# franciscotln/cosmology-model-fit

Hardware: AMD Instinct MI355X
Metric: walker-logL evals/s, Pantheon+ 1701-SN full-cov chi2, theta resident in HBM (higher is better)
Workload: dtype f64; 1 GPU; Pantheon+-shaped 1701-SN full-cov flat-LCDM chi2 + prior, 4096 walkers per GPU per step (BASELINE configs[1] at N=1), G=4000, theta resident in HBM; workload_key=pantheon, walkers_per_gpu=4096, walkers_total=4096, n_sn=1701, n_grid=4000, ndim=4, parallelism=walkers sharded over 1 GPU(s)

## Files before the change

cosmology-model-fit_amd/_lib.py:

```python
from __future__ import annotations

import ctypes as C
import os
import subprocess

_HERE = os.path.dirname(os.path.abspath(__file__))
LIB_PATH = os.environ.get("COSMOFIT_LIB") or os.path.join(_HERE, "libcosmofit_hip.so")
CSRC = os.path.join(_HERE, "csrc")

CF_ABI_VERSION = 11
CF_P_NSLOTS = 15
SLOTS = ("offset", "H0", "Om", "obh2", "och2", "w0", "wa", "v", "rd", "fcc", "lin", "v2", "v3", "s8", "fs8err")

CF_EZ_LATE_FLAT, CF_EZ_PHYSICAL = 0, 1
CF_FDE_LCDM, CF_FDE_WCDM, CF_FDE_THAWING, CF_FDE_CPL = 0, 1, 2, 3
CF_OUT_CHI2, CF_OUT_LOGL, CF_OUT_LOGP = 0, 1, 2
CF_SOLVE_BLOCKED_TRSM, CF_SOLVE_INVERSE_GEMM, CF_SOLVE_AUTO = 0, 1, 2
SOLVE_MODES = {"blocked": CF_SOLVE_BLOCKED_TRSM, "inverse": CF_SOLVE_INVERSE_GEMM, "auto": CF_SOLVE_AUTO}
CF_CMB_NONE = 0
STATUS = {0: "CF_OK", -1: "CF_ERR_INVALID", -2: "CF_ERR_NO_DEVICE", -3: "CF_ERR_HIP", -4: "CF_ERR_NOT_POSDEF",
          -5: "CF_ERR_UNSUPPORTED", -6: "CF_ERR_ILL_CONDITIONED"}


class CosmofitError(RuntimeError):
# ... 86 lines not shown
        ("qsr_offset", cf_param), ("qsr_scatter", cf_param),
        ("fde_n", C.c_double), ("fde_k", C.c_double), ("fde_p", C.c_double),
        ("qsr_z_top", C.c_double), ("sn_z_top", C.c_double),
        ("sn_zhel", C.c_int32), ("bao_mode", C.c_int32), ("n_bao", C.c_int32), ("_pad", C.c_int32),
        ("bao_z", C.c_void_p), ("bao_val", C.c_void_p), ("bao_qty", C.c_void_p), ("bao_inv_cov", C.c_void_p),
    ]


CF_DQ_MAX, CF_CURVE_MAX_NZ = 32, 4096
DERIVED_CODES = {"H0": 0, "h": 1, "Om": 2, "omh2": 3, "obh2": 4, "och2": 5, "w0": 6, "wa": 7, "q0": 8, "j0": 9, "S8": 10, "rd": 11,
                 "z_star": 12, "r_drag": 13, "z_drag": 14, "z_eq": 15, "H@": 16,
                 "rs_star": 32, "DM_star": 33, "theta_star100": 34, "R": 35, "lA": 36}
CURVE_CODES = {"H": 0, "DM": 1, "DV_rd": 2, "DM_rd": 3, "DH_rd": 4, "F_AP": 5, "mu": 6}


class cf_derived_consts(C.Structure):
    _fields_ = [("struct_size", C.c_int32), ("has_rdrag_fit", C.c_int32), ("zdrag_fit", C.c_double * 10),
                ("rdrag_fit", C.c_double * 11), ("zeq_or_h2", C.c_double)]


CF_GP_NDIM, CF_GP_MAX_N, CF_GP_MAX_NZ = 4, 64, 65536


class cf_gp_desc(C.Structure):
    _fields_ = [("struct_size", C.c_int32), ("device", C.c_int32), ("n", C.c_int32), ("_pad", C.c_int32),
                ("z", C.c_void_p), ("y", C.c_void_p), ("cov", C.c_void_p), ("bounds", C.c_void_p)]


class cf_gp_info(C.Structure):
    _fields_ = [("n", C.c_int32), ("device", C.c_int32), ("ld", C.c_int32), ("lds_bytes", C.c_int32),
                ("failed_factorizations", C.c_int64)]


CF_FIELD_MAX_NQ, CF_FIELD_MAX_NDIM, CF_FIELD_NPAR, CF_FIELD_NSCALAR, CF_FIELD_LAUNCH_ROWS = 4096, 64, 4, 5, 1 << 22
CF_FIELD_OK, CF_FIELD_PHANTOM, CF_FIELD_BAD = 0, 1, 2
FIELD_PARS = ("H0", "Om", "w0", "wa")
FIELD_SCALARS = ("phi_today", "t_today", "hubble_time", "phi_max", "t_max")
FIELD_OUTPUTS = ("phi_a", "t_a", "w_a", "K_a", "V_a", "phi_grid", "a_phi", "V_phi", "t_grid", "a_t", "phi_t")


class cf_field_desc(C.Structure):
    _fields_ = [("struct_size", C.c_int32), ("fde", C.c_int32), ("n_a", C.c_int32), ("ndim", C.c_int32), ("n_par", C.c_int32),
                ("_pad", C.c_int32), ("a_min", C.c_double), ("a_max", C.c_double), ("orh2", C.c_double),
                ("par", cf_param * CF_FIELD_NPAR)]


class cf_field_queries(C.Structure):
    _fields_ = [("a_q", C.c_void_p), ("phi_q", C.c_void_p), ("t_q", C.c_void_p), ("n_aq", C.c_int32), ("n_phi", C.c_int32),
                ("n_t", C.c_int32), ("_pad", C.c_int32)]


class cf_field_out(C.Structure):
    _fields_ = [(name, C.c_void_p) for name in FIELD_OUTPUTS + ("scalars", "status")]


CF_RB_SN, CF_RB_BAO = 0, 1
CF_RS_NCOL, CF_RESID_MAX_THR, CF_RESID_CHUNK = 10, 4, 4096
RESID_BLOCKS = {"sn": CF_RB_SN, "bao": CF_RB_BAO}
RESID_COLUMNS = ("mean", "std", "ss_res", "rmsd", "ss_tot", "r2", "skew", "kurtosis", "max_pull", "max_pull_index")
CHI2_BLOCK_COLUMNS = ("chi2_sn", "chi2_bao", "chi2_cmb", "cmb_v0", "cmb_v1", "cmb_v2", "chi2_cc", "chi2_fs8", "z_star", "r_drag")


class cf_resid_acc(C.Structure):
    _fields_ = [("struct_size", C.c_int32), ("n", C.c_int32), ("n_thr", C.c_int32), ("_pad", C.c_int32),
                ("w_sum", C.c_void_p), ("mean", C.c_void_p), ("m2", C.c_void_p), ("exceed", C.c_void_p),
                ("n_used", C.c_void_p), ("n_skipped", C.c_void_p)]


CF_MOCK_CHUNK = 4096


class cf_mock_set(C.Structure):
    _fields_ = [("struct_size", C.c_int32), ("n_mocks", C.c_int32), ("n_sn", C.c_int32), ("n_bao", C.c_int32),
                ("n_cmb", C.c_int32), ("_pad", C.c_int32),
                ("g_sn", C.c_void_p), ("g_bao", C.c_void_p), ("g_cmb", C.c_void_p), ("c", C.c_void_p)]


class cf_info(C.Structure):
    _fields_ = [
        ("n_sn", C.c_int64), ("n_sn_pad", C.c_int64), ("packed_chol_bytes", C.c_int64),
        ("workspace_bytes", C.c_int64), ("max_walkers", C.c_int64), ("nonfinite_count", C.c_int64),
        ("device", C.c_int32), ("cu_count", C.c_int32), ("gcn_arch", C.c_char * 64),
        ("pack_probe_rel", C.c_double), ("solve_mode", C.c_int32), ("n_devices", C.c_int32),
        ("devices", C.c_int32 * 16),
    ]


_VP, _I64, _I32 = C.c_void_p, C.c_int64, C.c_int32
EXPORTS = {
    "cf_device_count": (C.c_int, []),
    "cf_last_error": (C.c_char_p, []),
    "cf_abi_version": (C.c_int, []),
    "cf_create": (C.c_int, [C.POINTER(cf_desc), C.POINTER(_VP)]),
    "cf_destroy": (None, [_VP]),
    "cf_get_info": (C.c_int, [_VP, C.POINTER(cf_info)]),
    "cf_eval": (C.c_int, [_VP, _VP, _I64, _VP, _I32]),
    "cf_split_rows": (None, [_I64, _I32, _I32, C.POINTER(_I64), C.POINTER(_I64)]),
    "cf_eval_device": (C.c_int, [_VP, _VP, _I64, _VP, _I32, _VP]),
    "cf_eval_parts": (C.c_int, [_VP, _VP, _I64, _VP, _VP, _VP, _VP, _VP, _VP]),
    "cf_eval_table": (C.c_int, [_VP, _VP, _I64, _VP, _VP]),
    "cf_eval_bao_at": (C.c_int, [_VP, _VP, _VP, _VP, _I64, _VP]),
    "cf_eval_hz": (C.c_int, [_VP, _VP, _VP, _I64, _VP]),
    "cf_eval_fs8_at": (C.c_int, [_VP, _VP, _VP, _I64, _VP]),
    "cf_last_kernel_ms": (C.c_int, [_VP, C.POINTER(C.c_float * 2)]),
    "cf_enable_timing": (C.c_int, [_VP, C.c_int]),
    "cf_set_timing_stride": (C.c_int, [_VP, C.c_int]),
    "cf_timed_calls": (C.c_int64, [_VP]),
    "cf_kernel_ms": (C.c_int, [_VP, _I64, C.POINTER(C.c_float * 2)]),
    "cf_kernel_ms3": (C.c_int, [_VP, _I64, C.POINTER(C.c_float * 3)]),
    "cf_interp_hermite": (C.c_int, [_VP, _I64, _VP, _VP, _VP, _I64, _VP]),
    "cf_interp_pchip": (C.c_int, [_VP, _I64, _VP, _VP, _I64, _VP]),
    "cf_solve_triangular": (C.c_int, [_VP, _I64, _I64, _VP, _I64, _VP]),
    "cf_selftest_invpack_host": (C.c_int, [_VP, _I64, _I64, _VP, C.POINTER(C.c_double), C.POINTER(C.c_double)]),
    "cf_selftest_log10": (C.c_int, [_VP, _I64, _VP]),
    "cf_selftest_log10_tab": (C.c_int, [_VP, _I64, _VP]),
    "cf_selftest_exp_tab": (C.c_int, [_VP, _I64, _VP]),
    "cf_selftest_pos_ops": (C.c_int, [_VP, _VP, _I64, _VP]),
    "cf_ens_active_count": (_I64, [C.c_uint64, _I32, _I32, _I64, _I64]),
    "cf_ens_comp_count": (_I64, [C.c_uint64, _I32, _I32, _I64]),
    "cf_ens_active_set": (C.c_int, [C.c_uint64, _I32, _I32, _I64, _I64, _VP, _VP, _VP]),
    "cf_ens_kde_prepare": (C.c_int, [_VP, _I64, _I32, _I32, _I32, C.c_uint64, _VP, _VP, _VP]),
    "cf_ens_propose": (C.c_int, [_I32, _VP, _I64, _I32, _I32, _I32, C.c_uint64, _VP, _I64, C.c_uint64, C.c_double,
                                 C.c_double, _VP, _VP, _VP, _VP, _VP]),
    "cf_ens_accept": (C.c_int, [_VP, _VP, _I64, C.c_int32, C.c_uint64, _VP, _VP, _VP, _VP, _VP, _VP, _VP]),
    "cf_ens_accept_record": (C.c_int, [_VP, _VP, _I64, C.c_int32, C.c_uint64, _VP, _VP, _VP, _VP, _VP, _VP, _VP, _VP, _VP,
                                       _VP]),
    "cf_chain_mean": (C.c_int, [_VP, _I64, _I64, _VP, _VP]),
    "cf_chain_lagsum": (C.c_int, [_VP, _VP, _I64, _I64, _I64, _I32, _VP, _VP]),
    "cf_chain_acf_mean": (C.c_int, [_VP, _VP, _I64, _I32, _I32, _VP, _VP]),
    "cf_marg_bin": (C.c_int, [_VP, _I64, _I32, _VP, _I32, _VP, _VP]),
    "cf_marg_hist": (C.c_int, [_VP, _VP, C.c_double, _I64, _I32, _I32, _VP, _I32, _VP, _VP, _I32, _VP]),
    "cf_ns_prior_draw": (C.c_int, [_VP, _I64, C.c_uint64, _VP, _VP, _VP]),
    "cf_ns_transform": (C.c_int, [_VP, _VP, _I64, _VP, _VP]),
    "cf_ns_walk_start": (C.c_int, [_VP, _VP, _VP, _I64, _I32, _I64, C.c_uint64, _VP, _VP, _VP, _VP]),
    "cf_ns_propose": (C.c_int, [_VP, _VP, _I64, _I64, C.c_uint64, C.c_double, C.c_double, _VP, _VP, _VP, _VP, _VP, _VP]),
    "cf_ns_accept": (C.c_int, [_I64, _I32, _VP, _VP, _VP, _VP, _VP, _VP, _VP, _VP, _VP, _VP]),
    "cf_selftest_pack_host": (C.c_int, [_VP, _I64, _I64, _VP, C.POINTER(C.c_double), C.POINTER(_I64)]),
    "cf_create_quasar": (C.c_int, [C.POINTER(cf_desc), C.POINTER(cf_qsr_ext), C.POINTER(_VP)]),
    "cf_qsr_eval_parts": (C.c_int, [_VP, _VP, _I64, _VP, _VP, _VP, _VP]),
    "cf_opt_starts": (C.c_int, [C.POINTER(cf_opt_params), _I64, _VP, C.c_uint64, _I32, _VP, _VP, _VP]),
    "cf_opt_stencil": (C.c_int, [C.POINTER(cf_opt_params), C.POINTER(cf_opt_state), _VP, _I64, _VP, _VP]),
    "cf_opt_direction": (C.c_int, [C.POINTER(cf_opt_params), C.POINTER(cf_opt_state), _VP, _I64, _VP, _VP, _VP]),
    "cf_opt_accept": (C.c_int, [C.POINTER(cf_opt_params), C.POINTER(cf_opt_state), _VP, _I64, _VP, _VP]),
    "cf_opt_compact": (C.c_int, [_VP, _I64, _VP, _VP, _VP, _VP]),
    "cf_derived_device": (C.c_int, [_VP, _VP, _I64, _VP, _VP, _I32, _VP, _VP, _VP]),
    "cf_curves_device": (C.c_int, [_VP, _VP, _I64, _I32, _VP, _I32, _VP, _VP]),
    "cf_derived": (C.c_int, [_VP, _VP, _I64, _VP, _VP, _I32, _VP, _VP]),
    "cf_curves": (C.c_int, [_VP, _VP, _I64, _I32, _VP, _I32, _VP]),
    "cf_gp_create": (C.c_int, [C.POINTER(cf_gp_desc), C.POINTER(_VP)]),
    "cf_gp_destroy": (None, [_VP]),
    "cf_gp_get_info": (C.c_int, [_VP, C.POINTER(cf_gp_info)]),
    "cf_gp_mll_device": (C.c_int, [_VP, _VP, _I64, _VP, _VP, _VP]),
    "cf_gp_predict_device": (C.c_int, [_VP, _VP, _I64, _VP, _I32, C.c_double, _VP, _VP]),
    "cf_gp_mll": (C.c_int, [_VP, _VP, _I64, _VP, _VP]),
    "cf_gp_predict": (C.c_int, [_VP, _VP, _I64, _VP, _I32, C.c_double, _VP]),
    "cf_field_launch_count": (_I64, [_I64]),
    "cf_field_launch_range": (None, [_I64, _I64, C.POINTER(_I64), C.POINTER(_I64)]),
    "cf_field_device": (C.c_int, [C.POINTER(cf_field_desc), _VP, _I64, C.POINTER(cf_field_queries), C.POINTER(cf_field_out), _VP]),
    "cf_field": (C.c_int, [C.POINTER(cf_field_desc), _VP, _I64, C.POINTER(cf_field_queries), C.POINTER(cf_field_out)]),
    "cf_resid_device": (C.c_int, [_VP, _VP, _I64, _VP, _I32, _VP, _I32, _VP, _VP, C.POINTER(cf_resid_acc), _VP]),
    "cf_resid": (C.c_int, [_VP, _VP, _I64, _VP, _I32, _VP, _I32, _VP, _VP, C.POINTER(cf_resid_acc)]),
    "cf_resid_check_args": (C.c_int, [_I64, _I32, _I32, _I32, _VP, _I64, _I32, _VP, _I32, _VP, _VP, C.POINTER(cf_resid_acc)]),
    "cf_resid_sigma": (C.c_int, [_VP, _I32, _VP]),
    "cf_resid_set_chunk": (C.c_int, [_VP, _I64]),
    "cf_mock_eval_device": (C.c_int, [_VP, C.POINTER(cf_mock_set), _VP, _I64, _VP, _I32, _VP, _VP, _VP]),
    "cf_mock_eval": (C.c_int, [_VP, C.POINTER(cf_mock_set), _VP, _I64, _VP, _I32, _VP, _VP]),
    "cf_mock_check_args": (C.c_int, [_I64, _I32, _I32, _I32, _I32, C.POINTER(cf_mock_set), _VP, _I64, _VP, _I32, _VP]),
# ... 49 lines not shown
```

cosmology-model-fit_amd/csrc/cf_pack.h:

```cpp
#ifndef CF_PACK_H
#define CF_PACK_H

#include <cmath>
#include <cstdint>
#include <thread>
#include <vector>

#include "cosmofit_device.h"

struct cf_host_pack {
  int64_t n = 0, n_pad = 0;
  int32_t n_blocks = 0, ksplit = 1, tclasses = 4;
  std::vector<cf_d2> frags;
  std::vector<int64_t> upd_off;
  std::vector<int64_t> diag_off;
};

static inline int cf_tiles_in_block(int64_t T, int b) {
  int64_t left = T - (int64_t)b * CF_BLOCK_TILES;
  return (int)(left < CF_BLOCK_TILES ? left : CF_BLOCK_TILES);
}
static inline int cf_slots_of_wave(int tiles_b, int tq, int TC) { return tiles_b > tq ? (tiles_b - tq + TC - 1) / TC : 0; }

static inline int cf_diag_ml_max(int NW, int v, int tiles_b) {
// ... 221 lines not shown
  if (nt == 1) {
    work(0);
  } else {
    std::vector<std::thread> th;
    for (unsigned t = 0; t < nt; ++t) th.emplace_back(work, t);
    for (auto& x : th) x.join();
  }
}

static inline int64_t cf_inv_col(int64_t s2, int kq, int h) { return 8 * s2 + 2 * kq + h; }

static void cf_pack_inverse(const double* L, int64_t n, int64_t ld, cf_host_invpack& out) {
  const int64_t n_pad = (n + 15) / 16 * 16, T = n_pad / 16;
  const int RB = (int)((T + 3) / 4);
  out.n = n;
  out.n_pad = n_pad;
  out.n_rowblocks = RB;
  out.off.assign((size_t)RB * 4, 0);
  std::vector<double> X;
  cf_invert_lower(L, n, ld, n_pad, X);
  int64_t total = 0;
  for (int rb = 0; rb < RB; ++rb)
    for (int g = 0; g < 4; ++g) {
      out.off[rb * 4 + g] = total;
      total += (int64_t)2 * (rb + 1) * 4;
    }
  total += 32;
  out.frags.assign((size_t)total * 64, cf_d2{0.0, 0.0});
  for (int rb = 0; rb < RB; ++rb)
    for (int g = 0; g < 4; ++g) {
      cf_d2* st = out.frags.data() + out.off[rb * 4 + g] * 64;
      const int64_t nq = 2 * (rb + 1);
      for (int64_t q = 0; q < nq; ++q)
        for (int j = 0; j < 4; ++j)
          for (int lane = 0; lane < 64; ++lane) {
            const int64_t row = 64 * rb + 16 * j + (lane & 15);
            if (row >= n_pad) continue;
            const int64_t c0 = cf_inv_col(g * nq + q, lane >> 4, 0), c1 = cf_inv_col(g * nq + q, lane >> 4, 1);
            cf_d2& f = st[(q * 4 + j) * 64 + lane];
            f.x = c0 <= row ? X[(size_t)row * n_pad + c0] : 0.0;
            f.y = c1 <= row ? X[(size_t)row * n_pad + c1] : 0.0;
          }
    }
}

static double cf_invpack_replay_host(const cf_host_invpack& pk, const double* b_in) {
  const int64_t n_ld = (int64_t)pk.n_rowblocks * 64;
  std::vector<double> b((size_t)n_ld + 64, 0.0);
  for (int64_t i = 0; i < pk.n; ++i) b[i] = b_in[i];
  double chi = 0.0;
  for (int rb = 0; rb < pk.n_rowblocks; ++rb) {
    double y[64] = {0.0};
    const int64_t nq = 2 * (rb + 1);
    for (int g = 0; g < 4; ++g) {
      const cf_d2* st = pk.frags.data() + pk.off[rb * 4 + g] * 64;
      for (int64_t q = 0; q < nq; ++q)
        for (int j = 0; j < 4; ++j)
          for (int lane = 0; lane < 64; ++lane) {
            const cf_d2& f = st[(q * 4 + j) * 64 + lane];
            y[16 * j + (lane & 15)] += f.x * b[cf_inv_col(g * nq + q, lane >> 4, 0)] + f.y * b[cf_inv_col(g * nq + q, lane >> 4, 1)];
          }
    }
    for (int i = 0; i < 64; ++i) chi += y[i] * y[i];
  }
  return chi;
}

static double cf_invpack_probe(const cf_host_invpack& pk, const double* L, int64_t ld) {
  double worst = 0.0;
  for (int rb = 0; rb < pk.n_rowblocks; ++rb)
    for (int g = 0; g < 4; ++g)
      if (pk.off[rb * 4 + g] != cf_inv_stream_off(rb, g)) return INFINITY;
  std::vector<double> b;
  for (int mode = 0; mode < CF_PROBE_MODES; ++mode) {
    cf_probe_rhs(mode, pk.n, b);
    const double ref = cf_probe_reference(L, pk.n, ld, b);
    const double got = cf_invpack_replay_host(pk, b.data());
    const double rel = std::fabs(got - ref) / (std::fabs(ref) > 0 ? std::fabs(ref) : 1.0);
    if (!(rel <= worst)) worst = rel;
  }
  return worst;
}

#endif
```

cosmology-model-fit_amd/csrc/cosmofit_api.hip:

```cpp
#include <hip/hip_runtime.h>
#include <sys/prctl.h>

#include <cmath>
#include <cstdio>
#include <cstdlib>
#include <chrono>
#include <cstring>
#include <algorithm>
#include <atomic>
#include <utility>
#include <condition_variable>
#include <memory>
#include <mutex>
#include <string>
#include <thread>
#include <vector>

#include "../../include/cosmofit.h"
#include "cf_pack.h"
#include "cosmofit_device.h"
#include "cosmofit_mock.h"
#include "cosmofit_resid.h"

typedef double d2 __attribute__((ext_vector_type(2)));

#define CF_YPK_SLACK 8192
#define CF_DELTA_SLACK 4096

static long long cf_tune(const char* key, long long dflt) {
  static const std::string env = [] { const char* e = getenv("CF_TUNE"); return std::string(e ? e : ""); }();
  const size_t kl = strlen(key);
  for (size_t pos = 0; pos < env.size();) {
    const size_t end = std::min(env.find(',', pos), env.size());
    if (end - pos > kl + 1 && env.compare(pos, kl, key) == 0 && env[pos + kl] == '=') return atoll(env.c_str() + pos + kl + 1);
    pos = end + 1;
  }
  return dflt;
}

#define CF_BAO_NODES 6
#define CF_SN_PARTS_MAX 4
#define CF_SN_REC_SLACK (512 * CF_SN_PARTS_MAX)
template <int MODEL, int FDE>
__global__ void walker_kernel(cf_dev_desc d, const double* theta, int64_t W, double* delta, double* dm_out, double* mucorr_out,
                              d2* bao_nodes, d2* table_out);
template <int MODEL, int FDE>
__global__ void walker_fast_kernel(cf_walker_args d, const double* theta, int64_t W, double* delta, d2* bao_nodes, double* theta_copy,
                                   int frag_b, int sn_parts);
template <int MODEL, int FDE, int LANES, int ROLES>
__global__ void small_blocks_kernel(cf_dev_desc d, const double* theta, int64_t W, const d2* bao_nodes, double* chi2_extra,
                                    double* blocks_out, double* bao_out);
template <int MODEL, int FDE, int C>
__global__ void growth_kernel(cf_dev_desc d, const double* theta, int64_t W, const d2* aux_nodes, double* chi2_extra, int accumulate,
                              double* blocks_out, double* theory_out);
template <int MODEL, int FDE>
__global__ void hz_kernel(cf_dev_desc d, const double* theta, const double* z, int64_t n, double* out);
#define CF_DECLARE_GROWTH(M, F, C) \
  extern template __global__ void growth_kernel<M, F, C>(cf_dev_desc, const double*, int64_t, const d2*, double*, int, double*, double*);
#define CF_DECLARE_WALKER(M, F)                                                                                            \
  extern template __global__ void walker_kernel<M, F>(cf_dev_desc, const double*, int64_t, double*, double*, double*, d2*, d2*); \
  extern template __global__ void walker_fast_kernel<M, F>(cf_walker_args, const double*, int64_t, double*, d2*, double*, int, int); \
  extern template __global__ void small_blocks_kernel<M, F, 16, 1>(cf_dev_desc, const double*, int64_t, const d2*, double*, \
                                                                   double*, double*);                                      \
  extern template __global__ void small_blocks_kernel<M, F, 64, 1>(cf_dev_desc, const double*, int64_t, const d2*, double*, \
                                                                   double*, double*);                                      \
  extern template __global__ void small_blocks_kernel<M, F, 64, 2>(cf_dev_desc, const double*, int64_t, const d2*, double*, \
                                                                   double*, double*);                                      \
  extern template __global__ void hz_kernel<M, F>(cf_dev_desc, const double*, const double*, int64_t, double*);             \
  CF_DECLARE_GROWTH(M, F, 1) CF_DECLARE_GROWTH(M, F, 2) CF_DECLARE_GROWTH(M, F, 4) CF_DECLARE_GROWTH(M, F, 8)
CF_DECLARE_WALKER(0, 0) CF_DECLARE_WALKER(0, 1) CF_DECLARE_WALKER(0, 2) CF_DECLARE_WALKER(0, 3)
CF_DECLARE_WALKER(1, 0) CF_DECLARE_WALKER(1, 1) CF_DECLARE_WALKER(1, 2) CF_DECLARE_WALKER(1, 3)

typedef void (*walker_fn)(cf_dev_desc, const double*, int64_t, double*, double*, double*, d2*, d2*);
static walker_fn pick_walker(int model, int fde) {
  static const walker_fn table[2][4] = {
      {walker_kernel<0, 0>, walker_kernel<0, 1>, walker_kernel<0, 2>, walker_kernel<0, 3>},
      {walker_kernel<1, 0>, walker_kernel<1, 1>, walker_kernel<1, 2>, walker_kernel<1, 3>}};
  return table[model][fde];
}
typedef void (*walker_fast_fn)(cf_walker_args, const double*, int64_t, double*, d2*, double*, int, int);
static walker_fast_fn pick_walker_fast(int model, int fde) {
  static const walker_fast_fn table[2][4] = {
      {walker_fast_kernel<0, 0>, walker_fast_kernel<0, 1>, walker_fast_kernel<0, 2>, walker_fast_kernel<0, 3>},
      {walker_fast_kernel<1, 0>, walker_fast_kernel<1, 1>, walker_fast_kernel<1, 2>, walker_fast_kernel<1, 3>}};
  return table[model][fde];
}
static bool walker_fast_ok(const cf_dev_desc& d) {
  static const bool off = cf_tune("walker_generic", 0) != 0;
  return !off && d.chunk_shift == 3 && d.ndim <= 64 && !d.sn_fixed_mu && !d.sn_dir && !d.sn_vel_mult && (!d.sn_lin || d.lin_in_rec);
}
static cf_epilogue epilogue_of(const cf_dev_desc& d) {
  cf_epilogue e{};
  e.ndim = d.ndim; e.has_bounds = d.has_bounds; e.n_gauss = d.n_gauss; e.n_chi2_gauss = d.n_chi2_gauss;
  e.cpl_wall = d.cpl_wall; e.n_fs8 = d.n_fs8; e.n_cc = d.n_cc; e.cc_f_inverse = d.cc_f_inverse;
  e.log_norm = d.log_norm; e.logl_const = d.logl_const; e.cc_logdet = d.cc_logdet;
  e.w0 = d.slot[CF_P_W0_D]; e.wa = d.slot[CF_P_WA_D]; e.fs8err = d.slot[CF_P_FS8ERR_D]; e.fcc = d.slot[CF_P_FCC_D];
  for (int k = 0; k < CF_MAX_NDIM; ++k) { e.lo[k] = d.lo[k]; e.hi[k] = d.hi[k]; }
  for (int k = 0; k < CF_MAX_GAUSS; ++k) {
    e.gauss_idx[k] = d.gauss_idx[k]; e.gauss_mean[k] = d.gauss_mean[k]; e.gauss_sigma[k] = d.gauss_sigma[k];
    e.chi2_gauss_idx[k] = d.chi2_gauss_idx[k]; e.chi2_gauss_mean[k] = d.chi2_gauss_mean[k]; e.chi2_gauss_sigma[k] = d.chi2_gauss_sigma[k];
  }
  return e;
}
static cf_walker_args walker_args_of(const cf_dev_desc& d) {
  cf_walker_args a{};
  a.ndim = d.ndim; a.n_grid = d.n_grid; a.ez_model = d.ez_model; a.fde = d.fde;
  a.chunk_shift = d.chunk_shift; a.om_mode = d.om_mode;
  a.n_sn = d.n_sn; a.n_ld = d.n_ld;
  a.has_vstep = d.has_vstep; a.step_pm1 = d.step_pm1; a.lin_in_rec = d.lin_in_rec; a.n_aux = d.n_aux;
  a.z_max = d.z_max; a.step = d.step; a.c = d.c; a.inv_step = d.inv_step; a.inv_last = d.inv_last;
  a.or_h2 = d.or_h2; a.omnu_h2 = d.omnu_h2;
  for (int k = 0; k < CF_N_SLOTS; ++k) a.slot[k] = d.slot[k];
  a.sn_rec = d.sn_rec; a.log10_tab = d.log10_tab; a.nu_sw = d.nu_sw; a.ln_sw = d.ln_sw; a.exp2_tab = d.exp2_tab;
  a.bao_base = d.bao_base;
  return a;
}
typedef void (*small_blocks_fn)(cf_dev_desc, const double*, int64_t, const d2*, double*, double*, double*);
static small_blocks_fn pick_small_blocks(int model, int fde, int lanes, int roles = 1) {
#define CF_SB_TABLE(L, R)                                                                                                                \
  {{small_blocks_kernel<0, 0, L, R>, small_blocks_kernel<0, 1, L, R>, small_blocks_kernel<0, 2, L, R>, small_blocks_kernel<0, 3, L, R>}, \
   {small_blocks_kernel<1, 0, L, R>, small_blocks_kernel<1, 1, L, R>, small_blocks_kernel<1, 2, L, R>, small_blocks_kernel<1, 3, L, R>}}
  static const small_blocks_fn narrow[2][4] = CF_SB_TABLE(16, 1);
  static const small_blocks_fn wide[2][4] = CF_SB_TABLE(64, 1);
  static const small_blocks_fn wide2[2][4] = CF_SB_TABLE(64, 2);
#undef CF_SB_TABLE
  return lanes == 64 ? (roles == 2 ? wide2[model][fde] : wide[model][fde]) : narrow[model][fde];
}
typedef void (*hz_fn)(cf_dev_desc, const double*, const double*, int64_t, double*);
static hz_fn pick_hz(int model, int fde) {
  static const hz_fn table[2][4] = {{hz_kernel<0, 0>, hz_kernel<0, 1>, hz_kernel<0, 2>, hz_kernel<0, 3>},
                                    {hz_kernel<1, 0>, hz_kernel<1, 1>, hz_kernel<1, 2>, hz_kernel<1, 3>}};
  return table[model][fde];
}
typedef void (*growth_fn)(cf_dev_desc, const double*, int64_t, const d2*, double*, int, double*, double*);
#define CF_GROWTH_ROW(M, C) {growth_kernel<M, 0, C>, growth_kernel<M, 1, C>, growth_kernel<M, 2, C>, growth_kernel<M, 3, C>}
static growth_fn pick_growth(int model, int fde, int steps) {
  static const growth_fn table[4][2][4] = {{CF_GROWTH_ROW(0, 1), CF_GROWTH_ROW(1, 1)}, {CF_GROWTH_ROW(0, 2), CF_GROWTH_ROW(1, 2)},
                                           {CF_GROWTH_ROW(0, 4), CF_GROWTH_ROW(1, 4)}, {CF_GROWTH_ROW(0, 8), CF_GROWTH_ROW(1, 8)}};
  const int c = steps / 256;
  return table[c == 1 ? 0 : c == 2 ? 1 : c == 4 ? 2 : 3][model][fde];
}
template <int KS, int TC>
__global__ void trsm_chi2_kernel(const cf_epilogue* epi, int n_pad, int n_ld, int ndim, cf_dev_pack pk, const double* theta, int64_t W,
                                 const double* delta, d2* ypk, const double* chi2_extra, double* out, int out_kind,
                                 unsigned long long* nonfinite, double* chi2_sn_out);
extern template __global__ void trsm_chi2_kernel<2, 4>(const cf_epilogue*, int, int, int, cf_dev_pack, const double*, int64_t, const double*,
                                                       d2*, const double*, double*, int, unsigned long long*, double*);
template <int NP, int PF>
__global__ void tri_gemm_chi2_kernel(const cf_epilogue* epi, const d2* frags, int n_ld, int ndim, int n_rb, const double* theta, int64_t W,
                                     const double* delta, int64_t w_pad, double* partial, unsigned int* arrivals, const double* chi2_extra,
                                     double* out, int out_kind, unsigned long long* nonfinite, double* chi2_sn_out, int panels_per_group,
                                     int snake, int nt_last, int diag_skip, int split_levels, unsigned long long* done_flag,
                                     unsigned long long done_seq);
template <int PF, bool FRAG, int TPW>
__global__ void tri_gemm_small_kernel(const cf_epilogue* epi, const d2* frags, int n_ld, int ndim, int n_rb, const double* theta, int64_t W,
                                      const double* delta, double* partial4, unsigned int* arrivals, const double* chi2_extra, double* out,
                                      int out_kind, unsigned long long* nonfinite, double* chi2_sn_out, int units_pad,
                                      unsigned long long* done_flag, unsigned long long done_seq);
#define CF_DECLARE_TRIGEMM_SMALL(PF, FRAG, TPW)                                                                                          \
  extern template __global__ void tri_gemm_small_kernel<PF, FRAG, TPW>(const cf_epilogue*, const d2*, int, int, int, const double*, int64_t, \
                                                                       const double*, double*, unsigned int*, const double*, double*, int, \
                                                                       unsigned long long*, double*, int, unsigned long long*, unsigned long long);
CF_DECLARE_TRIGEMM_SMALL(16, true, 1)
CF_DECLARE_TRIGEMM_SMALL(16, false, 1)
CF_DECLARE_TRIGEMM_SMALL(8, true, 2)
CF_DECLARE_TRIGEMM_SMALL(8, false, 2)
#define CF_DECLARE_TRIGEMM(NP, PF)                                                                                                       \
  extern template __global__ void tri_gemm_chi2_kernel<NP, PF>(const cf_epilogue*, const d2*, int, int, int, const double*, int64_t,     \
// ... 129 lines not shown
struct cf_qsr_state;
int cf_qsr_prepare(const cf_desc* c, const cf_qsr_ext* e, int64_t n_ld, cf_qsr_state** out);
void cf_qsr_free(cf_qsr_state* q);
int64_t cf_qsr_n_qsr(const cf_qsr_state* q);
int32_t cf_qsr_n_bao(const cf_qsr_state* q);
void cf_qsr_set_outputs(cf_qsr_state* q, double* parts, double* mu_sn, double* mu_q, double* bao);
int cf_qsr_launch(const cf_qsr_state* q, const double* theta, int64_t W, double* delta, double* extra, int out_kind, double* th_copy,
                  hipStream_t st);

struct cf_worker {
  std::thread th;
  std::mutex m;
  std::condition_variable cv;
  bool has_job = false, done = false, quit = false;
  const double* theta = nullptr;
  double* out = nullptr;
  int64_t W = 0;
  int out_kind = 0, rc = 0;
  std::string err;
};

struct cf_handle {
  int device = 0;
  int solve_mode = 0;
  PinnedBuf stage_in, stage_out;
  InversePack ipack;
  DevBuf partial, arrivals;
  DevBuf partial4;
  DevBuf epi;
  cf_epilogue epi_host{};
  hipStream_t stream = nullptr;
  hipStream_t last_stream = nullptr;
  bool has_last = false;
  std::vector<hipEvent_t> ev;
  int timing_slots = 0, timing_stride = 1;
  int64_t timed_calls = 0, eval_calls = 0;
  cf_dev_desc d{};
  PackedFactor pack;
  DevBuf z_cmb, z_hel, obs, sn_step, sn_rec, log10_tab;
  DevBuf bao_z, bao_val, bao_inv_cov, bao_qty, gl_x, gl_w, fixed_mu, cc_z, cc_h, cc_inv_cov, nu_grid, ln_grid, nu_sw, ln_sw, exp2_tab, sn_lin, sn_dir;
  DevBuf theta, out, delta, ypk, chi2_extra, nonfinite;
  DevBuf fs8_z, fs8_val, fs8_inv_cov, fs8_fid, fs8_step_of, fs8_order, fs8_tab, fs8_pts;
  DevBuf bao_nodes, bao_base;
  PinnedBuf done_flags;
  unsigned long long done_seq = 0;
  int done_armed = 0;
  bool theta_on_host = false;
  bool has_small_blocks = false;
  bool has_growth = false;
  cf_qsr_state* qsr = nullptr;
  int64_t max_walkers = 0;
  double pack_probe_rel = 0.0;
  int cu_count = 0;
  char arch[64] = {0};
  std::vector<cf_handle*> peers;
  std::vector<std::unique_ptr<cf_worker>> workers;
  std::mutex mu;
  std::vector<double> sigma_sn_host, sigma_bao_host;
  DevBuf sigma_sn, sigma_bao, r_mc, r_bt, r_blk, r_snb, r_fsb;
  bool sigma_uploaded = false;
  int64_t resid_rows = 0, resid_chunk = 0;
  int64_t mock_chunk = 0;
};

extern "C" int cf_abi_version(void) { return CF_ABI_VERSION; }
extern "C" const char* cf_last_error(void) { return g_err.c_str(); }

extern "C" int cf_device_count(void) {
  int n = 0;
  if (hipGetDeviceCount(&n) != hipSuccess) return 0;
  return n;
}

static int32_t aux_node_base(const cf_dev_desc& d, double xi) {
  const int G = d.n_grid;
  int i = xi * d.inv_step >= (double)G ? G : (xi > 0.0 ? (int)(xi * d.inv_step) : 0);
  i = i > G - 2 ? G - 2 : (i < 0 ? 0 : i);
  if (i > 0 && (double)i * d.step >= xi) --i;
  if (i < G - 2 && (double)(i + 1) * d.step < xi) ++i;
  int b = i - 2;
  return b < 0 ? 0 : (b > G - CF_BAO_NODES ? G - CF_BAO_NODES : b);
}

static std::vector<double> swizzle_for_walker_threads(const std::vector<double>& table) {
  std::vector<double> out(8 * 512);
  const size_t n = table.size();
  for (int k = 0; k < 8; ++k)
    for (int t = 0; t < 512; ++t) out[(size_t)k * 512 + t] = table[std::min((size_t)(8 * t + k), n - 1)];
  return out;
}

static int upload_vec(DevBuf& b, const double* src, int64_t n) {
  if (b.ensure((size_t)n * 8)) return CF_ERR_HIP;
  HIP_TRY(hipMemcpy(b.p, src, (size_t)n * 8, hipMemcpyHostToDevice));
  return 0;
}

static int upload_log10_table(DevBuf& b) {
  cf_d2 t[64];
  for (int j = 0; j < 64; ++j) {
    const long double c = 0.5L * (1.0L + ((long double)j + 0.5L) / 64.0L);
    t[j].x = (double)(1.0L / c);
    t[j].y = (double)log10l(c);
  }
  if (b.ensure(sizeof(t))) return CF_ERR_HIP;
  HIP_TRY(hipMemcpy(b.p, t, sizeof(t), hipMemcpyHostToDevice));
  return 0;
}

static int upload_exp2_table(DevBuf& b) {
  double t[64];
  for (int j = 0; j < 64; ++j) t[j] = (double)exp2l((long double)j / 64.0L);
  return upload_vec(b, t, 64);
}

static int ensure_workspace(cf_handle* h, int64_t W) {
  const int64_t w_pad = (W + 31) / 32 * 32;
  if (!h->done_flags.p) {
    if (h->done_flags.ensure((size_t)CF_DONE_FLAGS * 8)) return CF_ERR_HIP;
    memset(h->done_flags.p, 0, (size_t)CF_DONE_FLAGS * 8);
  }
  if (w_pad <= h->max_walkers) return 0;
  HIP_TRY(hipDeviceSynchronize());
  const int64_t n_pad = h->d.n_pad > 0 ? h->d.n_pad : 16, n_ld = h->d.n_ld > 0 ? h->d.n_ld : 64;
  if (h->theta.ensure((size_t)w_pad * (h->d.ndim > 0 ? h->d.ndim : 1) * 8)) return CF_ERR_HIP;
  if (h->out.ensure((size_t)w_pad * 8)) return CF_ERR_HIP;
  if (h->stage_in.ensure((size_t)w_pad * (h->d.ndim > 0 ? h->d.ndim : 1) * 8)) return CF_ERR_HIP;
  if (h->stage_out.ensure((size_t)w_pad * 8)) return CF_ERR_HIP;
  if (h->chi2_extra.ensure((size_t)w_pad * 8)) return CF_ERR_HIP;
  if (h->d.n_aux > 0 && h->bao_nodes.ensure((size_t)w_pad * h->d.n_aux * CF_BAO_NODES * sizeof(d2))) return CF_ERR_HIP;
  if (h->d.n_sn > 0 && h->solve_mode == CF_SOLVE_INVERSE_GEMM) {
    if (h->partial.ensure((size_t)w_pad * h->ipack.dev.n_rowblocks * 8)) return CF_ERR_HIP;
    if (h->arrivals.ensure((size_t)(w_pad / 16) * 4)) return CF_ERR_HIP;
    if (h->partial4.ensure((size_t)CF_SMALL_MAX_PANELS * 4 * h->ipack.dev.n_rowblocks * 16 * 8)) return CF_ERR_HIP;
    HIP_TRY(hipMemsetAsync(h->arrivals.p, 0, (size_t)(w_pad / 16) * 4, h->stream));
  }
  if (h->d.n_sn > 0) {
    if (h->delta.ensure((size_t)w_pad * n_ld * 8 + CF_DELTA_SLACK)) return CF_ERR_HIP;
    HIP_TRY(hipMemsetAsync(h->delta.p, 0, (size_t)w_pad * n_ld * 8 + CF_DELTA_SLACK, h->stream));
    if (h->solve_mode == CF_SOLVE_BLOCKED_TRSM) {
      if (h->ypk.ensure((size_t)w_pad * n_pad * 8 + CF_YPK_SLACK)) return CF_ERR_HIP;
      HIP_TRY(hipMemsetAsync(h->ypk.p, 0, (size_t)w_pad * n_pad * 8 + CF_YPK_SLACK, h->stream));
    }
    HIP_TRY(hipStreamSynchronize(h->stream));
  }
  h->max_walkers = w_pad;
  return 0;
}

static int validate_desc(const cf_desc* c) {
  if (c->abi_version != CF_ABI_VERSION || c->struct_size != (int32_t)sizeof(cf_desc))
    return fail(CF_ERR_INVALID, "cf_create: descriptor ABI version / size mismatch (got version " +
                                    std::to_string(c->abi_version) + ", size " + std::to_string(c->struct_size) +
                                    ", expected " + std::to_string(CF_ABI_VERSION) + ", " +
                                    std::to_string(sizeof(cf_desc)) + ")");
  if (c->ndim < 1 || c->ndim > CF_MAX_NDIM) return fail(CF_ERR_INVALID, "cf_create: ndim must be in 1..16");
  if (c->n_grid < 4 || c->n_grid > 8192)
    return fail(CF_ERR_INVALID, "cf_create: n_grid must be in 4..8192 (the {cum_dm, dh} table must fit the 160 KB LDS)");
  if (!(c->z_max > 0.0) || !std::isfinite(c->z_max)) return fail(CF_ERR_INVALID, "cf_create: z_max must be > 0");
  if (!(c->c_km_s > 0.0)) return fail(CF_ERR_INVALID, "cf_create: c_km_s must be > 0");
  if (c->ez_model != CF_EZ_LATE_FLAT && c->ez_model != CF_EZ_PHYSICAL) return fail(CF_ERR_INVALID, "cf_create: bad ez_model");
  if (c->fde < CF_FDE_LCDM || c->fde > CF_FDE_CPL) return fail(CF_ERR_INVALID, "cf_create: bad fde");
  if (c->n_bao < 0 || c->n_bao > CF_MAX_BAO) return fail(CF_ERR_INVALID, "cf_create: n_bao must be in 0..64");
  if (c->n_bao > 0) {
    if (c->n_grid < CF_BAO_NODES) return fail(CF_ERR_INVALID, "cf_create: a BAO block needs n_grid >= 6");
    if (!c->bao_z || !c->bao_val || !c->bao_qty || !c->bao_inv_cov)
      return fail(CF_ERR_INVALID, "cf_create: BAO block arrays must not be null");
    for (int k = 0; k < c->n_bao; ++k)
      if (c->bao_qty[k] < CF_BAO_DV || c->bao_qty[k] > CF_BAO_FAP) return fail(CF_ERR_INVALID, "cf_create: bad bao_qty code");
    if (c->rd_mode != CF_RD_PARAM && c->rd_mode != CF_RD_FIT) return fail(CF_ERR_INVALID, "cf_create: bad rd_mode");
    if (c->bao_dh_mode != CF_BAO_DH_PCHIP && c->bao_dh_mode != CF_BAO_DH_EXACT)
      return fail(CF_ERR_INVALID, "cf_create: bad bao_dh_mode");
    if (c->bao_dh_mode == CF_BAO_DH_PCHIP && c->n_grid < 3) return fail(CF_ERR_INVALID, "cf_create: PCHIP needs >= 3 grid nodes");
  }
// ... 348 lines not shown
    if ((rc = upload_vec(h->bao_z, c->bao_z, c->n_bao))) return bail(rc);
    if ((rc = upload_vec(h->bao_val, c->bao_val, c->n_bao))) return bail(rc);
    if ((rc = upload_vec(h->bao_inv_cov, c->bao_inv_cov, (int64_t)c->n_bao * c->n_bao))) return bail(rc);
    if (h->bao_qty.ensure((size_t)c->n_bao * 4)) return bail(CF_ERR_HIP);
    if (hipMemcpy(h->bao_qty.p, c->bao_qty, (size_t)c->n_bao * 4, hipMemcpyHostToDevice) != hipSuccess)
      return bail(fail(CF_ERR_HIP, "hipMemcpy(bao_qty) failed"));
    d.bao_z = h->bao_z.as<const double>();
    d.bao_val = h->bao_val.as<const double>();
    d.bao_inv_cov = h->bao_inv_cov.as<const double>();
    d.bao_qty = h->bao_qty.as<const int32_t>();
    resid_bao_sigma(c->bao_inv_cov, c->n_bao, h->sigma_bao_host);
  }
  if (d.n_aux > 0) {
    std::vector<int32_t> base((size_t)d.n_aux);
    for (int k = 0; k < d.n_aux; ++k) base[k] = aux_node_base(d, k < c->n_bao ? c->bao_z[k] : c->fs8_z[k - c->n_bao]);
    if (h->bao_base.ensure(base.size() * 4)) return bail(CF_ERR_HIP);
    if (hipMemcpy(h->bao_base.p, base.data(), base.size() * 4, hipMemcpyHostToDevice) != hipSuccess)
      return bail(fail(CF_ERR_HIP, "hipMemcpy(bao_base) failed"));
    d.bao_base = h->bao_base.as<const int32_t>();
  }
  if (c->n_fs8 > 0) {
    int rc;
    const int n = c->n_fs8;
    if ((rc = upload_vec(h->fs8_z, c->fs8_z, n))) return bail(rc);
    if ((rc = upload_vec(h->fs8_val, c->fs8_val, n))) return bail(rc);
    if ((rc = upload_vec(h->fs8_inv_cov, c->fs8_inv_cov, (int64_t)n * n))) return bail(rc);
    if ((rc = upload_vec(h->fs8_fid, c->fs8_fid, n))) return bail(rc);
    d.fs8_z = h->fs8_z.as<const double>();
    d.fs8_val = h->fs8_val.as<const double>();
    d.fs8_inv_cov = h->fs8_inv_cov.as<const double>();
    d.fs8_fid = h->fs8_fid.as<const double>();
    const double x0 = std::log(c->fs8_a_init), hstep = -x0 / d.fs8_steps;
    std::vector<int32_t> step_of, order;
    std::vector<double> pts;
    fs8_points(d, c->fs8_z, n, step_of, order, pts);
    if (h->fs8_step_of.ensure((size_t)n * 4) || h->fs8_order.ensure((size_t)n * 4)) return bail(CF_ERR_HIP);
    if (hipMemcpy(h->fs8_step_of.p, step_of.data(), (size_t)n * 4, hipMemcpyHostToDevice) != hipSuccess ||
        hipMemcpy(h->fs8_order.p, order.data(), (size_t)n * 4, hipMemcpyHostToDevice) != hipSuccess)
      return bail(fail(CF_ERR_HIP, "hipMemcpy(fs8 order) failed"));
    d.fs8_step_of = h->fs8_step_of.as<const int32_t>();
    d.fs8_order = h->fs8_order.as<const int32_t>();
    const int npts = 2 * d.fs8_steps + 1;
    std::vector<double> tab((size_t)(2 * (d.fs8_steps / 256)) * 257 * 4, 0.0);
    for (int m = 0; m < npts; ++m) {
      const double a = m == npts - 1 ? 1.0 : std::exp(x0 + m * (0.5 * hstep)), zp1 = 1.0 / a;
      double nu = 0.0, dnu = 0.0;
      if (c->ez_model == CF_EZ_PHYSICAL) {
        const double r = c->nu_m0 / zp1, mz_sq = r * r;
        double ws = 0.0, num = 0.0, den = 0.0;
        for (int i = 0; i < 5; ++i) {
          const double f = std::sqrt(c->nu_qs_sq[i] + mz_sq);
          ws += f * c->nu_ws[i];
          num += c->nu_ws[i] / f;
          den += c->nu_ws[i] * f;
        }
        nu = zp1 * zp1 * zp1 * zp1 * ws / c->nu_rho0;
        const double w_nu = (1.0 / 3) - (1.0 / 3) * mz_sq * num / den;
        dnu = nu * 3 * (1.0 + w_nu) / zp1;
      }
      const int c2 = 2 * (d.fs8_steps / 256);
      const size_t at = (size_t)(m % c2) * 257 + (size_t)(m / c2);
      tab[4 * at] = a; tab[4 * at + 1] = zp1; tab[4 * at + 2] = nu; tab[4 * at + 3] = dnu;
    }
    if ((rc = upload_vec(h->fs8_tab, tab.data(), (int64_t)tab.size()))) return bail(rc);
    d.fs8_tab = h->fs8_tab.as<const double>();
    if ((rc = upload_vec(h->fs8_pts, pts.data(), (int64_t)pts.size()))) return bail(rc);
    d.fs8_pts = h->fs8_pts.as<const double>();
  }
  if (c->ez_model == CF_EZ_PHYSICAL) {
    std::vector<double> nu((size_t)c->n_grid);
    for (int g = 0; g < c->n_grid; ++g) {
      const double z = g == c->n_grid - 1 ? c->z_max : (double)g * d.step;
      const double zp1 = 1.0 + z, r = c->nu_m0 / zp1, mz_sq = r * r;
      const double ws = std::sqrt(c->nu_qs_sq[0] + mz_sq) * c->nu_ws[0] + std::sqrt(c->nu_qs_sq[1] + mz_sq) * c->nu_ws[1] +
                        std::sqrt(c->nu_qs_sq[2] + mz_sq) * c->nu_ws[2] + std::sqrt(c->nu_qs_sq[3] + mz_sq) * c->nu_ws[3] +
                        std::sqrt(c->nu_qs_sq[4] + mz_sq) * c->nu_ws[4];
      const double zp1_2 = zp1 * zp1;
      nu[g] = zp1_2 * zp1_2 * ws / c->nu_rho0;
    }
    int rc;
    if ((rc = upload_vec(h->nu_grid, nu.data(), c->n_grid))) return bail(rc);
    d.nu_grid = h->nu_grid.as<const double>();
    if (d.chunk_shift == 3) {
      const std::vector<double> sw = swizzle_for_walker_threads(nu);
      if ((rc = upload_vec(h->nu_sw, sw.data(), (int64_t)sw.size()))) return bail(rc);
      d.nu_sw = h->nu_sw.as<const double>();
    }
  }
  if (c->fde == CF_FDE_WCDM || c->fde == CF_FDE_CPL) {
    std::vector<double> ln((size_t)c->n_grid);
    for (int g = 0; g < c->n_grid; ++g) {
      const double z = g == c->n_grid - 1 ? c->z_max : (double)g * d.step;
      ln[g] = (double)log1pl((long double)z);
    }
    int rc;
    if ((rc = upload_vec(h->ln_grid, ln.data(), c->n_grid))) return bail(rc);
    d.ln_grid = h->ln_grid.as<const double>();
    if (d.chunk_shift == 3) {
      const std::vector<double> sw = swizzle_for_walker_threads(ln);
      if ((rc = upload_vec(h->ln_sw, sw.data(), (int64_t)sw.size()))) return bail(rc);
      d.ln_sw = h->ln_sw.as<const double>();
      if ((rc = upload_exp2_table(h->exp2_tab))) return bail(rc);
      d.exp2_tab = h->exp2_tab.as<const double>();
    }
  }
  if (c->cmb_mode != CF_CMB_NONE && (c->fde == CF_FDE_WCDM || c->fde == CF_FDE_CPL)) {
    int rc;
    if (!d.exp2_tab) {
      if ((rc = upload_exp2_table(h->exp2_tab))) return bail(rc);
      d.exp2_tab = h->exp2_tab.as<const double>();
    }
    if (!d.log10_tab) {
      if ((rc = upload_log10_table(h->log10_tab))) return bail(rc);
      d.log10_tab = h->log10_tab.p;
    }
  }
  if (c->n_cc > 0) {
    int rc;
    if ((rc = upload_vec(h->cc_z, c->cc_z, c->n_cc))) return bail(rc);
    if ((rc = upload_vec(h->cc_h, c->cc_h, c->n_cc))) return bail(rc);
    if ((rc = upload_vec(h->cc_inv_cov, c->cc_inv_cov, (int64_t)c->n_cc * c->n_cc))) return bail(rc);
    d.cc_z = h->cc_z.as<const double>();
    d.cc_h = h->cc_h.as<const double>();
    d.cc_inv_cov = h->cc_inv_cov.as<const double>();
  }
  if (c->n_sn > 0 && c->sn_fixed_mu) {
    int rc;
    if ((rc = upload_vec(h->fixed_mu, c->sn_fixed_mu, c->n_sn))) return bail(rc);
    d.sn_fixed_mu = h->fixed_mu.as<const double>();
  }
  if (c->n_sn > 0 && c->sn_lin_coef) {
    int rc;
    if ((rc = upload_vec(h->sn_lin, c->sn_lin_coef, c->n_sn))) return bail(rc);
    d.sn_lin = h->sn_lin.as<const double>();
  }
  if (c->n_sn > 0 && c->sn_dir) {
    int rc;
    if ((rc = upload_vec(h->sn_dir, c->sn_dir, 3 * c->n_sn))) return bail(rc);
    d.sn_dir = h->sn_dir.as<const double>();
  }
  if (c->cmb_mode != CF_CMB_NONE) {
    int rc;
    if ((rc = upload_vec(h->gl_x, c->gl_x, c->n_gl))) return bail(rc);
    if ((rc = upload_vec(h->gl_w, c->gl_w, c->n_gl))) return bail(rc);
    d.gl_x = h->gl_x.as<const double>();
    d.gl_w = h->gl_w.as<const double>();
  }
  if (h->nonfinite.ensure(8)) return bail(CF_ERR_HIP);
  if (hipMemset(h->nonfinite.p, 0, 8) != hipSuccess) return bail(fail(CF_ERR_HIP, "hipMemset failed"));
  if (d.chunk_shift == 3 && ((d.ez_model == CF_EZ_PHYSICAL_D && !d.nu_sw) ||
                             ((d.fde == CF_FDE_WCDM_D || d.fde == CF_FDE_CPL_D) && (!d.ln_sw || !d.exp2_tab))))
    return bail(fail(CF_ERR_INVALID, "cf_create: internal: the table build's neutrino / ln(1 + z) tables are missing"));
  h->epi_host = epilogue_of(d);
  if (h->epi.ensure(sizeof(cf_epilogue))) return bail(CF_ERR_HIP);
  if (hipMemcpy(h->epi.p, &h->epi_host, sizeof(cf_epilogue), hipMemcpyHostToDevice) != hipSuccess)
    return bail(fail(CF_ERR_HIP, "hipMemcpy of the epilogue block failed"));
  *out = h;
  return CF_OK;
}

static int eval_host_single(cf_handle* h, const double* theta, int64_t W, double* out, int out_kind, bool worker_thread = false);

static void worker_main(cf_handle* replica, cf_worker* w) {
  (void)hipSetDevice(replica->device);
  std::unique_lock<std::mutex> lk(w->m);
  for (;;) {
    w->cv.wait(lk, [&] { return w->has_job || w->quit; });
    if (w->quit) return;
    w->has_job = false;
    lk.unlock();
    const int rc = eval_host_single(replica, w->theta, w->W, w->out, w->out_kind, true);
    const std::string err = rc ? g_err : std::string();
    lk.lock();
    w->rc = rc;
    w->err = err;
    w->done = true;
    w->cv.notify_all();
  }
}

extern "C" int cf_create(const cf_desc* c, cf_handle** out) {
  if (!c || !out) return fail(CF_ERR_INVALID, "cf_create: null argument");
  *out = nullptr;
  int rc = validate_desc(c);
  if (rc) return rc;
  int ndev = 0;
  if (hipGetDeviceCount(&ndev) != hipSuccess || ndev == 0)
    return fail(CF_ERR_NO_DEVICE, "cf_create: no HIP device visible (this library has no CPU path)");
  std::vector<int> devs;
  if (c->n_devices == 0) devs.push_back(c->device);
  else if (c->n_devices < 0) for (int i = 0; i < ndev; ++i) devs.push_back(i);
  else devs.assign(c->devices, c->devices + c->n_devices);
  for (int dv : devs)
    if (dv < 0 || dv >= ndev) return fail(CF_ERR_INVALID, "cf_create: device ordinal out of range");
  HostPrep prep;
  cf_handle* primary = nullptr;
  if ((rc = create_one(c, devs[0], prep, &primary))) return rc;
  for (size_t k = 1; k < devs.size(); ++k) {
    cf_handle* r = nullptr;
    if ((rc = create_one(c, devs[k], prep, &r))) {
      const std::string keep = g_err;
      cf_destroy(primary);
      return fail(rc, keep);
    }
    primary->peers.push_back(r);
    primary->workers.emplace_back(new cf_worker());
    cf_worker* w = primary->workers.back().get();
    w->th = std::thread(worker_main, r, w);
  }
  *out = primary;
  return CF_OK;
}

extern "C" void cf_destroy(cf_handle* h) {
  if (!h) return;
  for (auto& w : h->workers) {
    {
      std::lock_guard<std::mutex> lk(w->m);
      w->quit = true;
    }
    w->cv.notify_all();
    if (w->th.joinable()) w->th.join();
  }
  for (cf_handle* r : h->peers) cf_destroy(r);
  DeviceScope on_device(h->device);
  (void)hipDeviceSynchronize();
  for (auto& e : h->ev)
    if (e) (void)hipEventDestroy(e);
  if (h->stream) (void)hipStreamDestroy(h->stream);
  cf_qsr_free(h->qsr);
  delete h;
}

extern "C" int cf_get_info(cf_handle* h, cf_info* info) {
  if (!h || !info) return fail(CF_ERR_INVALID, "cf_get_info: null argument");
  std::lock_guard<std::mutex> lk(h->mu);
  memset(info, 0, sizeof(*info));
  info->n_sn = h->d.n_sn;
  info->n_sn_pad = h->d.n_pad;
  info->packed_chol_bytes = h->pack.bytes + h->ipack.bytes;
  info->solve_mode = h->solve_mode;
  info->workspace_bytes = (int64_t)(h->theta.bytes + h->out.bytes + h->delta.bytes + h->ypk.bytes + h->partial.bytes +
                                    h->arrivals.bytes + h->bao_nodes.bytes + h->chi2_extra.bytes);
  info->max_walkers = h->max_walkers;
  info->device = h->device;
  info->cu_count = h->cu_count;
  info->pack_probe_rel = h->pack_probe_rel;
  info->n_devices = 1 + (int32_t)h->peers.size();
  info->devices[0] = h->device;
  for (size_t k = 0; k < h->peers.size() && k + 1 < 16; ++k) info->devices[k + 1] = h->peers[k]->device;
  snprintf(info->gcn_arch, sizeof(info->gcn_arch), "%s", h->arch);
  unsigned long long nf = 0;
  DeviceScope on_device(h->device);
  HIP_TRY(on_device.err);
  HIP_TRY(hipStreamSynchronize(h->stream));
  HIP_TRY(hipMemcpy(&nf, h->nonfinite.p, 8, hipMemcpyDeviceToHost));
  info->nonfinite_count = (int64_t)nf;
  return CF_OK;
}

extern "C" int cf_enable_timing(cf_handle* h, int slots) {
  if (!h) return fail(CF_ERR_INVALID, "cf_enable_timing: null handle");
  if (slots < 0 || slots > 4096) return fail(CF_ERR_INVALID, "cf_enable_timing: slots must be in 0..4096");
  std::lock_guard<std::mutex> lk(h->mu);
  DeviceScope on_device(h->device);
  HIP_TRY(on_device.err);
  while ((int)h->ev.size() < 4 * slots) {
    hipEvent_t e;
    HIP_TRY(hipEventCreate(&e));
    h->ev.push_back(e);
  }
  h->timing_slots = slots;
  h->timed_calls = 0;
  h->eval_calls = 0;
  return CF_OK;
}

extern "C" int cf_set_timing_stride(cf_handle* h, int stride) {
  if (!h || stride < 1) return fail(CF_ERR_INVALID, "cf_set_timing_stride: stride must be >= 1");
  std::lock_guard<std::mutex> lk(h->mu);
  h->timing_stride = stride;
  h->eval_calls = 0;
  return CF_OK;
}

extern "C" int64_t cf_timed_calls(cf_handle* h) { return h ? h->timed_calls : 0; }

extern "C" int cf_kernel_ms3(cf_handle* h, int64_t call, float t[3]) {
  if (!h || !t) return fail(CF_ERR_INVALID, "cf_kernel_ms3: null argument");
  if (h->timing_slots == 0 || call < 0 || call >= h->timed_calls || call < h->timed_calls - h->timing_slots)
    return fail(CF_ERR_INVALID, "cf_kernel_ms3: that call is not in the timing ring");
  const int slot = (int)(call % h->timing_slots);
  hipEvent_t* e = &h->ev[4 * slot];
  HIP_TRY(hipEventSynchronize(e[3]));
  for (int k = 0; k < 3; ++k) HIP_TRY(hipEventElapsedTime(&t[k], e[k], e[k + 1]));
  return CF_OK;
}

extern "C" int cf_kernel_ms(cf_handle* h, int64_t call, float t[2]) {
  float t3[3];
  if (!t) return fail(CF_ERR_INVALID, "cf_kernel_ms: null argument");
  const int rc = cf_kernel_ms3(h, call, t3);
  if (rc) return rc;
  t[0] = t3[0] + t3[1];
  t[1] = t3[2];
  return CF_OK;
}

extern "C" int cf_last_kernel_ms(cf_handle* h, float t[2]) {
  if (!h || !t) return fail(CF_ERR_INVALID, "cf_last_kernel_ms: null argument");
  if (h->timed_calls == 0) return fail(CF_ERR_INVALID, "cf_last_kernel_ms: call cf_enable_timing(h, slots>0) before evaluating");
  return cf_kernel_ms(h, h->timed_calls - 1, t);
}

static int launch_trsm(const cf_epilogue* epi, int n_pad, int n_ld, int ndim, const cf_dev_pack& pk, const double* d_theta, int64_t W,
                       const double* delta, d2* ypk, const double* chi2_extra, double* d_out, int out_kind, unsigned long long* nf,
                       hipStream_t st, double* chi2_sn_out = nullptr) {
  if (pk.ksplit != 2 || pk.tclasses != 4) return fail(CF_ERR_INVALID, "bad solve shape");
  const size_t lds = (size_t)2 * (CF_BLOCK_ROWS / 8 * 64) * sizeof(d2);
  static thread_local int attr_device = -1;
  int dev = 0;
  HIP_TRY(hipGetDevice(&dev));
  if (lds > 64 * 1024 && attr_device != dev) {
    HIP_TRY(hipFuncSetAttribute((const void*)(&trsm_chi2_kernel<2, 4>), hipFuncAttributeMaxDynamicSharedMemorySize, (int)lds));
    attr_device = dev;
  }
  const unsigned panels = (unsigned)((W + 15) / 16);
  hipLaunchKernelGGL((trsm_chi2_kernel<2, 4>), dim3(panels), dim3(512), lds, st, epi, n_pad, n_ld, ndim, pk, d_theta, W, delta, ypk, chi2_extra, d_out, out_kind, nf, chi2_sn_out);
  return 0;
}

// ... 33 lines not shown
  const int n_groups = (panels + ppg - 1) / ppg;
  static const int split_env = (int)cf_tune("gemm_split", -1);
  const int split_levels = NP == 2 ? std::max(0, std::min(a.n_rb - 1, split_env >= 0 ? split_env : (panels >= 28 && panels <= 56 ? 6 : 0))) : 0;
  const int n_wgs = n_groups * ppg * (a.n_rb + split_levels);
  static const int order_env = (int)cf_tune("gemm_order", -1);
  const int snake = order_env >= 0 ? order_env : (n_wgs <= 1024 + 256 ? 1 : 0);
  hipLaunchKernelGGL((tri_gemm_chi2_kernel<NP, PF>), dim3((unsigned)n_wgs), dim3(256), 0, st, a.epi, a.frags, a.n_ld, a.ndim, a.n_rb, a.theta,
                     a.W, a.delta, a.w_pad, a.partial, a.arrivals, a.chi2_extra, a.out, a.out_kind, a.nonfinite, a.chi2_sn_out, ppg, snake,
                     a.nt_last, a.diag_skip, split_levels, a.done_flag, a.done_seq);
  return 0;
}

template <int PF, bool FRAG, int TPW>
static int launch_tri_gemm_small_t(const TriGemmArgs& a, hipStream_t st) {
  const int panels = (int)((a.W + 15) / 16);
  const int units_pad = ((4 / TPW) * a.n_rb + 7) / 8 * 8;
  static const bool cap2 = cf_tune("small_lds_cap", 1) != 0;
  static const size_t static_lds = [] {
    hipFuncAttributes fa;
    return hipFuncGetAttributes(&fa, reinterpret_cast<const void*>(&tri_gemm_small_kernel<PF, FRAG, TPW>)) == hipSuccess ? fa.sharedSizeBytes
                                                                                                                          : (size_t)0;
  }();
  static const size_t cu_lds = [] {
    int dev = 0;
    hipDeviceProp_t pr;
    return (hipGetDevice(&dev) == hipSuccess && hipGetDeviceProperties(&pr, dev) == hipSuccess) ? (size_t)pr.maxSharedMemoryPerMultiProcessor
                                                                                                 : (size_t)0;
  }();
  size_t dyn_lds = 64 * a.n_rb <= 4096 ? (size_t)80 * a.n_rb * 8 : 0;
  const size_t third_of_cu = cu_lds / 3 + 1024;
  if (cap2 && static_lds > 0 && cu_lds > 0 && static_lds + dyn_lds < third_of_cu && third_of_cu <= 64 * 1024)
    dyn_lds = third_of_cu - static_lds;
  hipLaunchKernelGGL((tri_gemm_small_kernel<PF, FRAG, TPW>), dim3((unsigned)(panels * units_pad)), dim3(256), dyn_lds, st, a.epi, a.frags, a.n_ld,
                     a.ndim, a.n_rb, a.theta, a.W, a.delta, a.partial4, a.arrivals, a.chi2_extra, a.out, a.out_kind, a.nonfinite,
                     a.chi2_sn_out, units_pad, a.done_flag, a.done_seq);
  return 0;
}

static int64_t small_batch_max() {
  static const int64_t v = [] {
    const long long m = cf_tune("small_max", CF_SMALL_DEFAULT);
    return (int64_t)(m < 0 ? 0 : (m > 16 * CF_SMALL_MAX_PANELS ? 16 * CF_SMALL_MAX_PANELS : m));
  }();
  return v;
}

static int tri_gemm_panel_width(int64_t W) {
  static const int forced = (int)cf_tune("gemm_np", 0);
  return forced == 1 ? 16 : forced == 2 ? 32 : (W > CF_NP2_FROM ? 32 : 16);
}

static int launch_tri_gemm(const TriGemmArgs& a, hipStream_t st) {
  if (a.W <= small_batch_max() && a.partial4) {
    static const int tpw_env = (int)cf_tune("small_tpw", 0);
    const int tpw = (tpw_env == 1 || tpw_env == 2) ? tpw_env : (a.W <= 96 ? 1 : 2);
    if (tpw == 2) return a.frag_b ? launch_tri_gemm_small_t<8, true, 2>(a, st) : launch_tri_gemm_small_t<8, false, 2>(a, st);
    return a.frag_b ? launch_tri_gemm_small_t<16, true, 1>(a, st) : launch_tri_gemm_small_t<16, false, 1>(a, st);
  }
  if (a.frag_b) return fail(CF_ERR_INVALID, "internal: fragment-ordered residuals handed to the throughput solve kernel");
  return tri_gemm_panel_width(a.W) == 32 ? launch_tri_gemm_t<2, 2>(a, st) : launch_tri_gemm_t<1, 2>(a, st);
}

static int launch_eval(cf_handle* h, const double* th, int64_t Wc, double* out, int out_kind, hipStream_t st,
                       double* dm_out, double* mucorr_out, double* blocks_out, double* bao_out, double* chi2_sn_out,
                       hipEvent_t* ev, double* fs8_block_out = nullptr, double* fs8_theory_out = nullptr) {
  const cf_dev_desc& d = h->d;
  unsigned long long* nf = h->nonfinite.as<unsigned long long>();
  double* delta = h->delta.as<double>();
  d2* bao_nodes = h->bao_nodes.as<d2>();
  if (ev) HIP_TRY(hipEventRecord(ev[0], st));
  if (ev && !(h->d.n_sn > 0 || h->has_small_blocks || h->has_growth || h->qsr)) HIP_TRY(hipEventRecord(ev[1], st));
  const bool walker_work = d.n_sn > 0 || h->has_small_blocks || h->has_growth;
  double* extra = (h->has_small_blocks || h->has_growth || h->qsr) ? h->chi2_extra.as<double>() : nullptr;
  static const bool frag_env = cf_tune("small_frag", 1) != 0;
  const bool small_solve = d.n_sn > 0 && h->solve_mode == CF_SOLVE_INVERSE_GEMM && h->partial4.p && Wc <= small_batch_max();
  const bool frag_b = frag_env && small_solve && !dm_out && !mucorr_out && walker_fast_ok(d) && !h->qsr;
  if (h->qsr) {
    double* th_copy = h->theta_on_host ? h->theta.as<double>() : nullptr;
    int rc = cf_qsr_launch(h->qsr, th, Wc, delta, extra, out_kind, th_copy, st);
    if (rc) return rc;
    if (th_copy) th = th_copy;
    if (ev) HIP_TRY(hipEventRecord(ev[1], st));
  } else if (walker_work) {
    const size_t lds = ((size_t)d.n_grid + (d.n_grid >> d.chunk_shift) + 2) * 16;
    if (!dm_out && !mucorr_out && walker_fast_ok(d)) {
      double* th_copy = h->theta_on_host ? h->theta.as<double>() : nullptr;
      static const int parts_env = (int)cf_tune("sn_parts", 0);
      int sn_parts = parts_env > 0 ? parts_env : (Wc <= 64 ? 4 : (Wc <= 160 ? 2 : 1));
      if (sn_parts > CF_SN_PARTS_MAX || d.n_sn == 0) sn_parts = 1;
      hipLaunchKernelGGL(pick_walker_fast(d.ez_model, d.fde), dim3((unsigned)(Wc * sn_parts)), dim3(512), lds, st, walker_args_of(d), th,
                         Wc, delta, bao_nodes, th_copy, frag_b ? 1 : 0, sn_parts);
      if (th_copy) th = th_copy;
    } else
      hipLaunchKernelGGL(pick_walker(d.ez_model, d.fde), dim3((unsigned)Wc), dim3(512), lds, st, d, th, Wc, delta, dm_out, mucorr_out,
                         bao_nodes, (d2*)nullptr);
    if (ev) HIP_TRY(hipEventRecord(ev[1], st));
    if (h->has_small_blocks) {
      static const int64_t wide_max = cf_tune("sb_wide_max", 2048);
      static const int64_t roles_max = cf_tune("sb_roles_max", 2048);
      const int lanes = Wc <= wide_max ? 64 : 16, roles = (lanes == 64 && Wc <= roles_max) ? 2 : 1, per_wg = 256 / (lanes * roles);
      hipLaunchKernelGGL(pick_small_blocks(d.ez_model, d.fde, lanes, roles), dim3((unsigned)((Wc + per_wg - 1) / per_wg)), dim3(256), 0, st, d, th, Wc,
                         (const d2*)bao_nodes, extra, blocks_out, bao_out);
    }
    if (h->has_growth)
      hipLaunchKernelGGL(pick_growth(d.ez_model, d.fde, d.fs8_steps), dim3((unsigned)Wc), dim3(256),
                         (size_t)(2 * (d.fs8_steps + 1) + 16 + CF_MAX_FS8 + 2 + 256) * 8, st, d, th, Wc, (const d2*)bao_nodes, extra,
                         h->has_small_blocks ? 1 : 0, fs8_block_out, fs8_theory_out);
  }
  if (ev) HIP_TRY(hipEventRecord(ev[2], st));
  if (d.n_sn > 0 && h->solve_mode == CF_SOLVE_INVERSE_GEMM) {
    static const bool trim = cf_tune("gemm_trim", 1) != 0;
    const int n_rb_ = h->ipack.dev.n_rowblocks, nt_last = trim ? std::max(1, std::min(4, (d.n_pad - 64 * (n_rb_ - 1)) / 16)) : 4;
    static const int diag_skip = cf_tune("gemm_diag_skip", 1) != 0;
    TriGemmArgs a{h->epi.as<const cf_epilogue>(), h->ipack.dev.frags, d.n_ld, d.ndim, n_rb_, nt_last, diag_skip, th, Wc, delta,
                  h->max_walkers, h->partial.as<double>(), h->arrivals.as<unsigned int>(), extra, out,
                  out_kind, nf, chi2_sn_out, h->partial4.as<double>(), nullptr, 0ull, frag_b};
    if (h->theta_on_host && h->done_flags.p) {
      a.done_flag = (unsigned long long*)h->done_flags.p;
      a.done_seq = h->done_seq;
      const bool small = Wc <= small_batch_max() && a.partial4;
      const int pw = small ? 16 : tri_gemm_panel_width(Wc);
      h->done_armed = (int)((Wc + pw - 1) / pw);
      if (h->done_armed > CF_DONE_FLAGS) { a.done_flag = nullptr; h->done_armed = 0; }
    }
    int rc = launch_tri_gemm(a, st);
    if (rc) return rc;
  } else if (d.n_sn > 0) {
    int rc = launch_trsm(h->epi.as<const cf_epilogue>(), d.n_pad, d.n_ld, d.ndim, h->pack.dev, th, Wc, delta, h->ypk.as<d2>(), extra, out,
                         out_kind, nf, st, chi2_sn_out);
    if (rc) return rc;
  } else {
    unsigned long long* fin_flag = nullptr;
    if (h->theta_on_host && h->done_flags.p && (Wc + 255) / 256 <= CF_DONE_FLAGS) {
      fin_flag = (unsigned long long*)h->done_flags.p;
      h->done_armed = (int)((Wc + 255) / 256);
    }
    hipLaunchKernelGGL(finalize_kernel, dim3((unsigned)((Wc + 255) / 256)), dim3(256), 0, st, h->epi_host, th, Wc, (const double*)extra, out,
                       out_kind, nf, fin_flag, h->done_seq);
  }
  if (ev) HIP_TRY(hipEventRecord(ev[3], st));
  return 0;
}

static int order_behind_last(cf_handle* h, hipStream_t st) {
  if (!h->has_last || h->last_stream == st) return 0;
  if (h->last_stream == h->stream)
    HIP_TRY(hipStreamSynchronize(h->stream));
  else
    HIP_TRY(hipDeviceSynchronize());
  h->has_last = false;
  return 0;
}

static int launch_path(cf_handle* h, const double* d_theta, int64_t W, double* d_out, int out_kind, hipStream_t st,
                       double* dm_out, double* mucorr_out, double* blocks_out, double* bao_out,
                       double* chi2_sn_out = nullptr, double* fs8_block_out = nullptr, double* fs8_theory_out = nullptr) {
  { int rc0 = order_behind_last(h, st); if (rc0) return rc0; }
  const bool timed = h->timing_slots && (h->eval_calls++ % h->timing_stride) == 0;
  const int slot = timed ? (int)(h->timed_calls % h->timing_slots) : 0;
  hipEvent_t* ev = timed ? &h->ev[4 * slot] : nullptr;
  int rc = launch_eval(h, d_theta, W, d_out, out_kind, st, dm_out, mucorr_out, blocks_out, bao_out, chi2_sn_out, ev, fs8_block_out,
                       fs8_theory_out);
  if (rc) return rc;
  if (ev) h->timed_calls++;
  h->last_stream = st;
  h->has_last = true;
  HIP_TRY(hipGetLastError());
  return 0;
}

static int check_eval_args(cf_handle* h, const void* theta, int64_t W, const void* out, int out_kind, const char* fn) {
  if (!h || !theta || !out) return fail(CF_ERR_INVALID, std::string(fn) + ": null argument");
  if (W < 0 || W > ((int64_t)1 << 24)) return fail(CF_ERR_INVALID, std::string(fn) + ": W out of range");
  if (out_kind < CF_OUT_CHI2 || out_kind > CF_OUT_LOGP) return fail(CF_ERR_INVALID, std::string(fn) + ": bad out_kind");
  return 0;
}

// ... 116 lines not shown
    w->cv.wait(lk, [&] { return w->done; });
    if (w->rc && !rc) {
      rc = w->rc;
      err = w->err;
    }
  }
  return rc ? fail(rc, err) : CF_OK;
}

extern "C" int cf_eval_parts(cf_handle* h, const double* theta, int64_t W, double* dm_obs, double* mu_corr,
                             double* delta, double* chi2_blocks, double* bao_theory, double* fs8_theory) {
  if (!h || !theta) return fail(CF_ERR_INVALID, "cf_eval_parts: null argument");
  if (h->qsr) return fail(CF_ERR_UNSUPPORTED, "cf_eval_parts: a quasar handle; use cf_qsr_eval_parts");
  if (W <= 0 || W > (1 << 20)) return fail(CF_ERR_INVALID, "cf_eval_parts: W out of range");
  if (bao_theory && h->d.n_bao == 0) return fail(CF_ERR_INVALID, "cf_eval_parts: this likelihood has no BAO block");
  if (fs8_theory && h->d.n_fs8 == 0) return fail(CF_ERR_INVALID, "cf_eval_parts: this likelihood has no growth-rate block");
  if ((dm_obs || mu_corr || delta) && h->d.n_sn == 0) return fail(CF_ERR_INVALID, "cf_eval_parts: this likelihood has no SN block");
  std::lock_guard<std::mutex> lk(h->mu);
  DeviceScope on_device(h->device);
  HIP_TRY(on_device.err);
  int rc;
  if ((rc = ensure_workspace(h, W))) return rc;
  const int64_t n = h->d.n_sn, n_ld = h->d.n_ld, nb = h->d.n_bao, nf = h->d.n_fs8;
  DevBuf dm, mc, blk, bt, snb, fsb, ft;
  if (snb.ensure((size_t)W * 8) || fsb.ensure((size_t)W * 8)) return CF_ERR_HIP;
  HIP_TRY(hipMemsetAsync(snb.p, 0, (size_t)W * 8, h->stream));
  HIP_TRY(hipMemsetAsync(fsb.p, 0, (size_t)W * 8, h->stream));
  if (n > 0 && dm.ensure((size_t)W * n * 8)) return CF_ERR_HIP;
  if (n > 0 && mu_corr && mc.ensure((size_t)W * n * 8)) return CF_ERR_HIP;
  if (blk.ensure((size_t)W * 8 * 8)) return CF_ERR_HIP;
  HIP_TRY(hipMemsetAsync(blk.p, 0, (size_t)W * 8 * 8, h->stream));
  if (nb > 0 && bt.ensure((size_t)W * nb * 8)) return CF_ERR_HIP;
  if (nf > 0 && ft.ensure((size_t)W * nf * 8)) return CF_ERR_HIP;
  HIP_TRY(hipMemcpyAsync(h->theta.p, theta, (size_t)W * h->d.ndim * 8, hipMemcpyHostToDevice, h->stream));
  if ((rc = launch_path(h, h->theta.as<const double>(), W, h->out.as<double>(), CF_OUT_CHI2, h->stream,
                        dm.as<double>(), mc.as<double>(), blk.as<double>(), bt.as<double>(), snb.as<double>(), fsb.as<double>(),
                        ft.as<double>())))
    return rc;
  HIP_TRY(hipStreamSynchronize(h->stream));
  if (dm_obs) HIP_TRY(hipMemcpy(dm_obs, dm.p, (size_t)W * n * 8, hipMemcpyDeviceToHost));
  if (mu_corr) HIP_TRY(hipMemcpy(mu_corr, mc.p, (size_t)W * n * 8, hipMemcpyDeviceToHost));
  if (delta && n > 0)
    HIP_TRY(hipMemcpy2D(delta, (size_t)n * 8, h->delta.p, (size_t)n_ld * 8, (size_t)n * 8, (size_t)W,
                        hipMemcpyDeviceToHost));
  if (bao_theory) HIP_TRY(hipMemcpy(bao_theory, bt.p, (size_t)W * nb * 8, hipMemcpyDeviceToHost));
  if (fs8_theory) HIP_TRY(hipMemcpy(fs8_theory, ft.p, (size_t)W * nf * 8, hipMemcpyDeviceToHost));
  if (chi2_blocks) {
    std::vector<double> sn((size_t)W), b8((size_t)W * 8), fs((size_t)W);
    HIP_TRY(hipMemcpy(sn.data(), snb.p, (size_t)W * 8, hipMemcpyDeviceToHost));
    HIP_TRY(hipMemcpy(b8.data(), blk.p, (size_t)W * 8 * 8, hipMemcpyDeviceToHost));
    HIP_TRY(hipMemcpy(fs.data(), fsb.p, (size_t)W * 8, hipMemcpyDeviceToHost));
    for (int64_t w = 0; w < W; ++w) {
      double* o = chi2_blocks + 10 * w;
      const double* b = &b8[8 * (size_t)w];
      o[0] = sn[w];
      o[1] = b[0]; o[2] = b[1]; o[3] = b[2]; o[4] = b[3]; o[5] = b[4]; o[6] = b[5];
      o[7] = fs[w];
      o[8] = b[6]; o[9] = b[7];
    }
  }
  return CF_OK;
}

extern "C" int cf_eval_table(cf_handle* h, const double* theta, int64_t W, double* cum_dm, double* dh) {
  if (!h || !theta || !cum_dm || !dh) return fail(CF_ERR_INVALID, "cf_eval_table: null argument");
  if (h->qsr) return fail(CF_ERR_UNSUPPORTED, "cf_eval_table: a quasar handle; use cf_qsr_eval_parts");
  if (W <= 0 || W > 4096) return fail(CF_ERR_INVALID, "cf_eval_table: W must be in 1..4096");
  std::lock_guard<std::mutex> lk(h->mu);
  DeviceScope on_device(h->device);
  HIP_TRY(on_device.err);
  int rc;
  if ((rc = ensure_workspace(h, W))) return rc;
  if ((rc = order_behind_last(h, h->stream))) return rc;
  cf_dev_desc d = h->d;
  const int G = d.n_grid;
  d.n_sn = 0;
  d.n_bao = 0;
  d.n_fs8 = 0;
  d.n_aux = 0;
  d.n_ld = 0;
  DevBuf tab;
  if (tab.ensure((size_t)W * G * sizeof(d2))) return CF_ERR_HIP;
  HIP_TRY(hipMemcpyAsync(h->theta.p, theta, (size_t)W * d.ndim * 8, hipMemcpyHostToDevice, h->stream));
  const size_t lds = ((size_t)G + (G >> d.chunk_shift) + 2) * 16;
  hipLaunchKernelGGL(pick_walker(d.ez_model, d.fde), dim3((unsigned)W), dim3(512), lds, h->stream, d, h->theta.as<const double>(), W,
                     (double*)nullptr, (double*)nullptr, (double*)nullptr, (d2*)nullptr, tab.as<d2>());
  HIP_TRY(hipGetLastError());
  std::vector<cf_d2> host((size_t)W * G);
  HIP_TRY(hipMemcpyAsync(host.data(), tab.p, host.size() * sizeof(cf_d2), hipMemcpyDeviceToHost, h->stream));
  HIP_TRY(hipStreamSynchronize(h->stream));
  for (size_t i = 0; i < host.size(); ++i) {
    cum_dm[i] = host[i].x;
    dh[i] = host[i].y;
  }
  return CF_OK;
}

extern "C" int cf_eval_fs8_at(cf_handle* h, const double* theta, const double* z, int64_t n, double* out) {
  if (!h || !theta || (n > 0 && (!z || !out))) return fail(CF_ERR_INVALID, "cf_eval_fs8_at: null argument");
  if (n < 0) return fail(CF_ERR_INVALID, "cf_eval_fs8_at: n must be >= 0");
  if (!h->has_growth) return fail(CF_ERR_INVALID, "cf_eval_fs8_at: the handle has no growth-rate block");
  for (int64_t k = 0; k < n; ++k)
    if (!(z[k] >= 0.0) || !(1.0 / (1.0 + z[k]) >= h->d.fs8_a_init))
      return fail(CF_ERR_INVALID, "cf_eval_fs8_at: redshifts must lie in a_init <= a <= 1");
  if (n == 0) return CF_OK;
  std::lock_guard<std::mutex> lk(h->mu);
  DeviceScope on_device(h->device);
  HIP_TRY(on_device.err);
  int rc;
  if ((rc = ensure_workspace(h, 1))) return rc;
  if ((rc = order_behind_last(h, h->stream))) return rc;
  HIP_TRY(hipMemcpyAsync(h->theta.p, theta, (size_t)h->d.ndim * 8, hipMemcpyHostToDevice, h->stream));
  const int B = CF_MAX_FS8;
  DevBuf dz, dbase, dstep, dorder, dpts, dval, dinv, dfid, nodes, dout, extra;
  if (dz.ensure(B * 8) || dbase.ensure(B * 4) || dstep.ensure(B * 4) || dorder.ensure(B * 4) || dpts.ensure(B * CF_FS8_REC * 8) ||
      dval.ensure(B * 8) || dinv.ensure((size_t)B * B * 8) || dfid.ensure(B * 8) ||
      nodes.ensure((size_t)B * CF_BAO_NODES * sizeof(d2)) || dout.ensure(B * 8) || extra.ensure(64))
    return CF_ERR_HIP;
  HIP_TRY(hipMemsetAsync(dval.p, 0, B * 8, h->stream));
  HIP_TRY(hipMemsetAsync(dinv.p, 0, (size_t)B * B * 8, h->stream));
  const std::vector<double> ones((size_t)B, 1.0);
  HIP_TRY(hipMemcpyAsync(dfid.p, ones.data(), B * 8, hipMemcpyHostToDevice, h->stream));
  for (int64_t k0 = 0; k0 < n; k0 += B) {
    const int m = (int)(n - k0 < B ? n - k0 : B);
    cf_dev_desc d = h->d;
    d.n_sn = 0; d.n_ld = 0; d.n_bao = 0; d.n_cc = 0; d.cmb_mode = 0;
    d.n_fs8 = m; d.n_aux = m;
    std::vector<int32_t> step_of, order, base((size_t)m);
    std::vector<double> pts;
    fs8_points(d, z + k0, m, step_of, order, pts);
    for (int k = 0; k < m; ++k) base[k] = aux_node_base(d, z[k0 + k]);
    HIP_TRY(hipMemcpyAsync(dz.p, z + k0, (size_t)m * 8, hipMemcpyHostToDevice, h->stream));
    HIP_TRY(hipMemcpyAsync(dbase.p, base.data(), (size_t)m * 4, hipMemcpyHostToDevice, h->stream));
    HIP_TRY(hipMemcpyAsync(dstep.p, step_of.data(), (size_t)m * 4, hipMemcpyHostToDevice, h->stream));
    HIP_TRY(hipMemcpyAsync(dorder.p, order.data(), (size_t)m * 4, hipMemcpyHostToDevice, h->stream));
    HIP_TRY(hipMemcpyAsync(dpts.p, pts.data(), (size_t)m * CF_FS8_REC * 8, hipMemcpyHostToDevice, h->stream));
    d.fs8_z = dz.as<const double>(); d.bao_base = dbase.as<const int32_t>(); d.fs8_step_of = dstep.as<const int32_t>();
    d.fs8_order = dorder.as<const int32_t>(); d.fs8_pts = dpts.as<const double>(); d.fs8_val = dval.as<const double>();
    d.fs8_inv_cov = dinv.as<const double>(); d.fs8_fid = dfid.as<const double>();
    const size_t lds = ((size_t)d.n_grid + (d.n_grid >> d.chunk_shift) + 2) * 16;
    hipLaunchKernelGGL(pick_walker(d.ez_model, d.fde), dim3(1), dim3(512), lds, h->stream, d, h->theta.as<const double>(), (int64_t)1,
                       (double*)nullptr, (double*)nullptr, (double*)nullptr, nodes.as<d2>(), (d2*)nullptr);
    hipLaunchKernelGGL(pick_growth(d.ez_model, d.fde, d.fs8_steps), dim3(1), dim3(256),
                       (size_t)(2 * (d.fs8_steps + 1) + 16 + CF_MAX_FS8 + 2 + 256) * 8, h->stream, d, h->theta.as<const double>(),
                       (int64_t)1, (const d2*)nodes.as<d2>(), extra.as<double>(), 0, (double*)nullptr, dout.as<double>());
    HIP_TRY(hipGetLastError());
    HIP_TRY(hipMemcpyAsync(out + k0, dout.p, (size_t)m * 8, hipMemcpyDeviceToHost, h->stream));
    HIP_TRY(hipStreamSynchronize(h->stream));
  }
  return CF_OK;
}

extern "C" int cf_eval_hz(cf_handle* h, const double* theta, const double* z, int64_t n, double* out) {
  if (!h || !theta || (n > 0 && (!z || !out))) return fail(CF_ERR_INVALID, "cf_eval_hz: null argument");
  if (h->qsr) return fail(CF_ERR_UNSUPPORTED, "cf_eval_hz: a quasar handle; use cf_qsr_eval_parts");
  if (n < 0) return fail(CF_ERR_INVALID, "cf_eval_hz: n must be >= 0");
  if (n == 0) return CF_OK;
  std::lock_guard<std::mutex> lk(h->mu);
  DeviceScope on_device(h->device);
  HIP_TRY(on_device.err);
  int rc;
  if ((rc = ensure_workspace(h, 1))) return rc;
  if ((rc = order_behind_last(h, h->stream))) return rc;
  DevBuf dz, dout;
  if (dz.ensure((size_t)n * 8) || dout.ensure((size_t)n * 8)) return CF_ERR_HIP;
  HIP_TRY(hipMemcpyAsync(h->theta.p, theta, (size_t)h->d.ndim * 8, hipMemcpyHostToDevice, h->stream));
  HIP_TRY(hipMemcpyAsync(dz.p, z, (size_t)n * 8, hipMemcpyHostToDevice, h->stream));
  hipLaunchKernelGGL(pick_hz(h->d.ez_model, h->d.fde), dim3((unsigned)((n + 255) / 256)), dim3(256), 0, h->stream, h->d,
                     h->theta.as<const double>(), dz.as<const double>(), n, dout.as<double>());
  HIP_TRY(hipGetLastError());
  HIP_TRY(hipMemcpyAsync(out, dout.p, (size_t)n * 8, hipMemcpyDeviceToHost, h->stream));
  HIP_TRY(hipStreamSynchronize(h->stream));
  return CF_OK;
}

extern "C" int cf_eval_bao_at(cf_handle* h, const double* theta, const double* z, const int32_t* qty, int64_t n, double* out) {
  if (!h || !theta || (n > 0 && (!z || !qty || !out))) return fail(CF_ERR_INVALID, "cf_eval_bao_at: null argument");
  if (h->qsr) return fail(CF_ERR_UNSUPPORTED, "cf_eval_bao_at: a quasar handle; use cf_qsr_eval_parts");
  if (n < 0) return fail(CF_ERR_INVALID, "cf_eval_bao_at: n must be >= 0");
  for (int64_t k = 0; k < n; ++k) {
    if (!std::isfinite(z[k])) return fail(CF_ERR_INVALID, "cf_eval_bao_at: z must be finite");
    if (qty[k] < 0 || qty[k] > 3) return fail(CF_ERR_INVALID, "cf_eval_bao_at: qty must be 0 (D_V), 1 (D_M), 2 (D_H) or 3 (F_AP)");
  }
  if (n == 0) return CF_OK;
  std::lock_guard<std::mutex> lk(h->mu);
  DeviceScope on_device(h->device);
  HIP_TRY(on_device.err);
  int rc;
  if ((rc = ensure_workspace(h, 1))) return rc;
  if ((rc = order_behind_last(h, h->stream))) return rc;
  HIP_TRY(hipMemcpyAsync(h->theta.p, theta, (size_t)h->d.ndim * 8, hipMemcpyHostToDevice, h->stream));
  DevBuf dz, dq, dbase, dval, dinv, nodes, dout, extra;
  const int B = CF_MAX_BAO;
  if (dz.ensure(B * 8) || dq.ensure(B * 4) || dbase.ensure(B * 4) || dval.ensure(B * 8) || dinv.ensure((size_t)B * B * 8) ||
      nodes.ensure((size_t)B * CF_BAO_NODES * sizeof(d2)) || dout.ensure(B * 8) || extra.ensure(64))
    return CF_ERR_HIP;
  HIP_TRY(hipMemsetAsync(dval.p, 0, B * 8, h->stream));
  HIP_TRY(hipMemsetAsync(dinv.p, 0, (size_t)B * B * 8, h->stream));
  for (int64_t k0 = 0; k0 < n; k0 += B) {
    const int m = (int)(n - k0 < B ? n - k0 : B);
    cf_dev_desc d = h->d;
    d.n_sn = 0; d.n_ld = 0; d.n_fs8 = 0; d.n_cc = 0; d.cmb_mode = 0;
    d.n_bao = m; d.n_aux = m;
    std::vector<int32_t> base((size_t)m);
    for (int k = 0; k < m; ++k) base[k] = aux_node_base(d, z[k0 + k]);
    HIP_TRY(hipMemcpyAsync(dz.p, z + k0, (size_t)m * 8, hipMemcpyHostToDevice, h->stream));
    HIP_TRY(hipMemcpyAsync(dq.p, qty + k0, (size_t)m * 4, hipMemcpyHostToDevice, h->stream));
    HIP_TRY(hipMemcpyAsync(dbase.p, base.data(), (size_t)m * 4, hipMemcpyHostToDevice, h->stream));
    d.bao_z = dz.as<const double>(); d.bao_qty = dq.as<const int32_t>(); d.bao_base = dbase.as<const int32_t>();
    d.bao_val = dval.as<const double>(); d.bao_inv_cov = dinv.as<const double>();
    const size_t lds = ((size_t)d.n_grid + (d.n_grid >> d.chunk_shift) + 2) * 16;
    hipLaunchKernelGGL(pick_walker(d.ez_model, d.fde), dim3(1), dim3(512), lds, h->stream, d, h->theta.as<const double>(), (int64_t)1,
                       (double*)nullptr, (double*)nullptr, (double*)nullptr, nodes.as<d2>(), (d2*)nullptr);
    hipLaunchKernelGGL(pick_small_blocks(d.ez_model, d.fde, 16), dim3(1), dim3(256), 0, h->stream, d, h->theta.as<const double>(), (int64_t)1,
                       (const d2*)nodes.as<d2>(), extra.as<double>(), (double*)nullptr, dout.as<double>());
    HIP_TRY(hipGetLastError());
    HIP_TRY(hipMemcpyAsync(out + k0, dout.p, (size_t)m * 8, hipMemcpyDeviceToHost, h->stream));
    HIP_TRY(hipStreamSynchronize(h->stream));
  }
  return CF_OK;
}

static int interp_common(const double* xq, int64_t nq, const double* x, const double* y, const double* yp, int64_t n,
                         double* out, int mode) {
  if (!xq || !x || !y || !out || (mode == 0 && !yp)) return fail(CF_ERR_INVALID, "cf_interp: null argument");
  if (nq < 0 || n < 2) return fail(CF_ERR_INVALID, "cf_interp: need n >= 2 nodes");
  if (mode == 1 && n < 3) return fail(CF_ERR_INVALID, "cf_interp_pchip: need n >= 3 nodes");
  if (cf_device_count() == 0) return fail(CF_ERR_NO_DEVICE, "cf_interp: no HIP device visible (this library has no CPU path)");
  if (nq == 0) return CF_OK;
  DevBuf dxq, dx, dy, dyp, dout;
  if (dxq.ensure((size_t)nq * 8) || dx.ensure((size_t)n * 8) || dy.ensure((size_t)n * 8) || dout.ensure((size_t)nq * 8))
    return CF_ERR_HIP;
  HIP_TRY(hipMemcpy(dxq.p, xq, (size_t)nq * 8, hipMemcpyHostToDevice));
  HIP_TRY(hipMemcpy(dx.p, x, (size_t)n * 8, hipMemcpyHostToDevice));
  HIP_TRY(hipMemcpy(dy.p, y, (size_t)n * 8, hipMemcpyHostToDevice));
  if (mode == 0) {
    if (dyp.ensure((size_t)n * 8)) return CF_ERR_HIP;
    HIP_TRY(hipMemcpy(dyp.p, yp, (size_t)n * 8, hipMemcpyHostToDevice));
  }
  hipLaunchKernelGGL(interp_kernel, dim3((unsigned)((nq + 255) / 256)), dim3(256), 0, 0, dxq.as<const double>(), nq,
                     dx.as<const double>(), dy.as<const double>(), dyp.as<const double>(), n, dout.as<double>(), mode);
  HIP_TRY(hipGetLastError());
  HIP_TRY(hipMemcpy(out, dout.p, (size_t)nq * 8, hipMemcpyDeviceToHost));
  return CF_OK;
}

extern "C" int cf_interp_hermite(const double* xq, int64_t nq, const double* x, const double* y, const double* y_prime,
                                 int64_t n, double* out) {
  return interp_common(xq, nq, x, y, y_prime, n, out, 0);
}

extern "C" int cf_interp_pchip(const double* xq, int64_t nq, const double* x, const double* y, int64_t n, double* out) {
  return interp_common(xq, nq, x, y, nullptr, n, out, 1);
}

extern "C" int cf_solve_triangular(const double* L, int64_t n, int64_t ld, const double* b, int64_t nrhs, double* out) {
  if (!L || !b || !out) return fail(CF_ERR_INVALID, "cf_solve_triangular: null argument");
  if (n < 1 || ld < n || nrhs < 0 || n > (1 << 20)) return fail(CF_ERR_INVALID, "cf_solve_triangular: bad sizes");
  if (cf_device_count() == 0)
    return fail(CF_ERR_NO_DEVICE, "cf_solve_triangular: no HIP device visible (this library has no CPU path)");
  if (nrhs == 0) return CF_OK;
  cf_host_pack hp;
  double probe = 0.0;
  if (pack_default(L, n, ld, hp, &probe) != 0)
    return fail(CF_ERR_NOT_POSDEF, "cf_solve_triangular: non-positive or non-finite diagonal entry");
  if (!(probe <= CF_PROBE_LIMIT))
    return fail(CF_ERR_ILL_CONDITIONED, "cf_solve_triangular: blocked solve loses " + std::to_string(probe) + " relative on this factor");
  PackedFactor pf;
  int rc;
  if ((rc = pf.upload(hp))) return rc;
  const int64_t w_pad = (nrhs + 15) / 16 * 16, n_pad = hp.n_pad, n_ld = (n + 63) / 64 * 64;
  DevBuf db, delta, ypk, dout, nf, dth, epi0;
  if (db.ensure((size_t)nrhs * n * 8) || delta.ensure((size_t)w_pad * n_ld * 8) || ypk.ensure((size_t)w_pad * n_pad * 8 + CF_YPK_SLACK) ||
      dout.ensure((size_t)w_pad * 8) || nf.ensure(8) || dth.ensure(8) || epi0.ensure(sizeof(cf_epilogue)))
    return CF_ERR_HIP;
  HIP_TRY(hipMemset(epi0.p, 0, sizeof(cf_epilogue)));
  HIP_TRY(hipMemcpy(db.p, b, (size_t)nrhs * n * 8, hipMemcpyHostToDevice));
  HIP_TRY(hipMemset(nf.p, 0, 8));
  hipLaunchKernelGGL(pad_rhs_kernel, dim3((unsigned)w_pad), dim3(256), 0, 0, db.as<const double>(), nrhs, n, n_ld,
                     delta.as<double>());
  if ((rc = launch_trsm(epi0.as<const cf_epilogue>(), (int)n_pad, (int)n_ld, 0, pf.dev, dth.as<const double>(), nrhs, delta.as<const double>(), ypk.as<d2>(), nullptr,
                        dout.as<double>(), (int)CF_OUT_CHI2, nf.as<unsigned long long>(), (hipStream_t)0, nullptr)))
    return rc;
  HIP_TRY(hipGetLastError());
  HIP_TRY(hipMemcpy(out, dout.p, (size_t)nrhs * 8, hipMemcpyDeviceToHost));
  return CF_OK;
}

extern "C" int cf_selftest_invpack_host(const double* L, int64_t n, int64_t ld, const double* b, double* chi2_out,
                                        double* probe_out) {
  if (!L || !b || !chi2_out) return fail(CF_ERR_INVALID, "cf_selftest_invpack_host: null argument");
  for (int64_t i = 0; i < n; ++i)
    if (!(L[i * ld + i] > 0.0) || !std::isfinite(L[i * ld + i])) return fail(CF_ERR_NOT_POSDEF, "cf_selftest_invpack_host: bad pivot");
  cf_host_invpack ip;
  cf_pack_inverse(L, n, ld, ip);
// ... 666 lines not shown
```

cosmology-model-fit_amd/csrc/cosmofit_kernels.hip:

```cpp
#include <hip/hip_runtime.h>
#include <type_traits>
#include <stdint.h>

#include "cosmofit_device.h"
#include "cf_wave_scan.h"

typedef double d4 __attribute__((ext_vector_type(4)));
typedef double d2 __attribute__((ext_vector_type(2)));

#define CF_WAVE 64

__device__ __forceinline__ double slot_get(const cf_dev_desc& d, int s, const double* __restrict__ th) {
  const cf_dev_slot& p = d.slot[s];
  return p.idx >= 0 ? p.scale * th[p.idx] : p.fixed;
}

struct ThetaRow {
  double v;
};
__device__ __forceinline__ double readlane_f64(double v, int lane) {
  return __hiloint2double(__builtin_amdgcn_readlane(__double2hiint(v), lane), __builtin_amdgcn_readlane(__double2loint(v), lane));
}
template <class D>
__device__ __forceinline__ double slot_get(const D& d, int s, const ThetaRow& th) {
// ... 142 lines not shown
  r = fma(fma(-b, r, 1.0), r, r);
  r = fma(fma(-b, r, 1.0), r, r);
  const double q = a * r;
  return fma(fma(-b, q, a), r, q);
}

__device__ __forceinline__ double grid_z(int i, int G, double step, double z_max) {
  return i == G - 1 ? z_max : (double)i * step;
}

template <int MODEL, int FDE>
__device__ __forceinline__ double dh_of_node(const cf_dev_desc& d, const WalkerCosmo& wc, double c_over_H0, int g) {
  const double nu = (MODEL == CF_EZ_PHYSICAL_D && d.nu_grid) ? d.nu_grid[g] : -1.0;
  return c_over_H0 * rsqrt(e2_of_z<MODEL, FDE>(d, wc, grid_z(g, d.n_grid, d.step, d.z_max), nu));
}

#define CF_TPB_A 512

struct DistTable {
  const d2* tab;
  int G, chs;
  double step, inv_step, inv_last, z_max;
  __device__ __forceinline__ d2 at(int g) const { return tab[g + (g >> chs)]; }
};

#define CF_BAO_NODES 6
struct NodeView {
  const d2* p;
  int base, G;
  double step, inv_step, inv_last, z_max;
  __device__ __forceinline__ d2 at(int g) const {
    int o = g - base;
    o = o < 0 ? 0 : (o > CF_BAO_NODES - 1 ? CF_BAO_NODES - 1 : o);
    return p[o];
  }
};

template <class TAB>
__device__ __forceinline__ double hermite_tab(const TAB& T, double xi) {
  const int G = T.G;
  if (xi <= 0.0) {
    const d2 e = T.at(0);
    return e.x + e.y * (xi - 0.0);
  }
  if (xi >= T.z_max) {
    const d2 e = T.at(G - 1);
    return e.x + e.y * (xi - T.z_max);
  }
  int i = (int)(xi * T.inv_step);
  i = i > G - 2 ? G - 2 : i;
  double x0 = (double)i * T.step;
  if (x0 >= xi) {
    --i;
    x0 = (double)i * T.step;
  }
  double x1 = grid_z(i + 1, G, T.step, T.z_max);
  if (x1 < xi) {
    ++i;
    x0 = x1;
    x1 = grid_z(i + 1, G, T.step, T.z_max);
  }
  const double h_i = x1 - x0;
  const double t = (xi - x0) * (i == G - 2 ? T.inv_last : T.inv_step);
  const double t2 = t * t, t3 = t2 * t;
  const double h00 = 2 * t3 - 3 * t2 + 1;
  const double h10 = t3 - 2 * t2 + t;
  const double h01 = -2 * t3 + 3 * t2;
  const double h11 = t3 - t2;
  const d2 e0 = T.at(i), e1 = T.at(i + 1);
  return h00 * e0.x + h10 * h_i * e0.y + h01 * e1.x + h11 * h_i * e1.y;
}

__device__ __forceinline__ double fma_vvs(double a, double b, double c_uniform) {
  double r;
  asm("v_fma_f64 %0, %1, %2, %3" : "=v"(r) : "v"(a), "v"(b), "s"(c_uniform));
  return r;
}
__device__ __forceinline__ double fma_vsv(double a, double b_uniform, double c) {
  double r;
  asm("v_fma_f64 %0, %1, %2, %3" : "=v"(r) : "v"(a), "s"(b_uniform), "v"(c));
  return r;
}

__device__ __forceinline__ double hermite_fast(const DistTable& T, double xi) {
  const int G = T.G;
  if (__builtin_expect(xi > 0.0 && xi < T.z_max, 1)) {
    const double u = xi * T.inv_step;
    int i = (int)u;
    i = i > G - 2 ? G - 2 : i;
    const double t = u - (double)i;
    const d2* p = T.tab + (i + (i >> T.chs));
    const d2 e0 = p[0], e1 = p[1];
    const double b = T.step * e0.y, hm1 = T.step * e1.y, dy = e1.x - e0.x;
    const double sm = b + hm1;
    const double dd = fma(-2.0, dy, sm);
    const double cc = fma(3.0, dy, -(sm + b));
    return fma(t, fma(t, fma(t, dd, cc), b), e0.x);
  }
  if (xi <= 0.0) {
    const d2 e = T.at(0);
    return e.x + e.y * xi;
  }
  const d2 e = T.at(G - 1);
  return e.x + e.y * (xi - T.z_max);
}

__device__ __forceinline__ double log10_pos(double x) {
  if (!(x > 2.2250738585072014e-308 && x < 1.7976931348623157e308)) return log10(x);
  const double ivln10hi = 4.34294481878168880939e-01, ivln10lo = 2.50829467116452752298e-11;
  const double log10_2hi = 3.01029995663611771306e-01, log10_2lo = 3.69423907715893078616e-13;
  const double Lg1 = 6.666666666666735130e-01, Lg2 = 3.999999999940941908e-01, Lg3 = 2.857142874366239149e-01,
               Lg4 = 2.222219843214978396e-01, Lg5 = 1.818357216161805012e-01, Lg6 = 1.531383769920937332e-01,
               Lg7 = 1.479819860511658591e-01;
  int k;
  double m = frexp(x, &k);
  if (m < 0.70710678118654752440) {
    m *= 2.0;
    k -= 1;
  }
  const double f = m - 1.0;
  const double hfsq = 0.5 * f * f;
  const double den = 2.0 + f;
  double r = __builtin_amdgcn_rcp(den);
  r = fma(fma(-den, r, 1.0), r, r);
  double sq = f * r;
  sq = fma(fma(-den, sq, f), r, sq);
  const double z = sq * sq, w = z * z;
  const double t1 = w * (Lg2 + w * (Lg4 + w * Lg6));
  const double t2 = z * (Lg1 + w * (Lg3 + w * (Lg5 + w * Lg7)));
  const double R = sq * (hfsq + (t2 + t1));
  double hi = f - hfsq;
  hi = __longlong_as_double(__double_as_longlong(hi) & 0xFFFFFFFF00000000ll);
  const double lo = (f - hi) - hfsq + R;
  double val_hi = hi * ivln10hi;
  const double dk = (double)k;
  const double y2 = dk * log10_2hi;
  double val_lo = dk * log10_2lo + (lo + hi) * ivln10lo + lo * ivln10hi;
  const double ww = y2 + val_hi;
  val_lo += (y2 - ww) + val_hi;
  return val_lo + ww;
}

__device__ __forceinline__ double log10_tab(double x, const d2* __restrict__ tab) {
  if (!(x > 2.2250738585072014e-308 && x < 1.7976931348623157e308)) return log10(x);
  const double C1 = 4.34294481903251827651e-01, C2 = -2.17147240951625913826e-01, C3 = 1.44764827301083942550e-01,
               C4 = -1.08573620475812956913e-01, C5 = 8.68588963806503655303e-02, C6 = -7.23824136505419712752e-02,
               C7 = 6.20420688433216896645e-02, C8 = -5.42868102379064784564e-02;
  const double log10_2hi = 3.01029995663611771306e-01, log10_2lo = 3.69423907715893078616e-13;
  const int e = __builtin_amdgcn_frexp_exp(x);
  const double m = __builtin_amdgcn_frexp_mant(x);
  const d2 t = tab[(__double2hiint(m) >> 14) & 63];
  const double r = fma(m, t.x, -1.0);
  double p = fma_vsv(r, C8, C7);
  p = fma_vvs(p, r, C6);
  p = fma_vvs(p, r, C5);
  p = fma_vvs(p, r, C4);
  p = fma_vvs(p, r, C3);
  p = fma_vvs(p, r, C2);
  p = fma_vvs(p, r, C1);
  const double ek = (double)e;
  return fma_vsv(ek, log10_2hi, t.y) + fma(r, p, ek * log10_2lo);
}


template <int MODEL, int FDE, int CH, bool LAST, class D>
__device__ __forceinline__ double chunk_eval(const D& d, const WalkerCosmo& wc, double c_over_H0, int g0, int lane,
                                             const double (&nu_pre)[CH], const double (&ln)[CH], const double* __restrict__ etab,
                                             double (&dh)[CH], double (&loc)[CH]) {
  const int G = d.n_grid;
  constexpr bool POWER_LAW = FDE == CF_FDE_WCDM_D || FDE == CF_FDE_CPL_D;
  double fde[CH];
  if (POWER_LAW) {
    double x[CH];
#pragma unroll
    for (int k = 0; k < CH; ++k) {
      const int g = g0 + k;
      double z = (double)g * d.step;
      if (LAST) z = g >= G - 1 ? d.z_max : z;
      if (FDE == CF_FDE_CPL_D) {
        const double zp1 = 1.0 + z;
        double r = __builtin_amdgcn_rcp(zp1);
        r = fma(fma(-zp1, r, 1.0), r, r);
        x[k] = fma(3 * (1 + wc.w0 + wc.wa), ln[k], (-3 * wc.wa) * (z * r));
      } else {
        x[k] = 3 * (1 + wc.w0) * ln[k];
      }
    }
    fde[0] = exp_tab(x[0], etab);
    double dx_max = 0.0;
#pragma unroll
    for (int k = 1; k < CH; ++k) {
      const double dx = x[k] - x[k - 1];
      dx_max = fmax(dx_max, fabs(dx));
      double p = fma(dx, 1.0 / 5040, 1.0 / 720);
      p = fma(p, dx, 1.0 / 120);
      p = fma(p, dx, 1.0 / 24);
      p = fma(p, dx, 1.0 / 6);
      p = fma(p, dx, 0.5);
      p = fma(p * dx, dx, dx);
      fde[k] = fma(fde[k - 1], p, fde[k - 1]);
    }
    if (!(dx_max < 0x1p-5)) {
#pragma unroll
      for (int k = 1; k < CH; ++k) fde[k] = exp_tab(x[k], etab);
    }
  }
#pragma unroll
  for (int k = 0; k < CH; ++k) {
    const int g = g0 + k;
    double z = (double)g * d.step;
    if (LAST) z = g >= G - 1 ? d.z_max : z;
    const double e2 = POWER_LAW ? e2_from_fde<MODEL>(wc, z, fde[k], nu_pre[k]) : e2_of_z<MODEL, FDE, true, D>(d, wc, z, nu_pre[k], ln[k], etab);
    const double v = c_over_H0 * rsqrt_pos(e2);
    dh[k] = (LAST && g >= G) ? 0.0 : v;
  }
  double prev = dpp_move<0x138, 0xF>(dh[CH - 1]);
  double run = 0.0;
  const double half = 0.5 * d.step;
#pragma unroll
  for (int k = 0; k < CH; ++k) {
    const bool counts = (k > 0 || lane > 0) && (!LAST || g0 + k < G);
    run = counts ? fma_vsv(prev + dh[k], half, run) : run;
    loc[k] = run;
    prev = dh[k];
  }
  return run;
}

template <int MODEL, int FDE, int CH, class D>
__device__ __forceinline__ void build_distance_table_regs(const D& d, const WalkerCosmo& wc, d2* tab,
                                                          d4* wave_pub, const double (&nu_pre)[CH], const double (&ln_pre)[CH],
                                                          const double* __restrict__ etab) {
  const int G = d.n_grid;
  const int tid = threadIdx.x, lane = tid & 63, wave = tid >> 6;
  const int g0 = tid * CH;
  const int base = g0 + tid;
  const double c_over_H0 = wc.c / wc.H0;
  double dh[CH], loc[CH];
  const int wave_last = (tid - lane) * CH + 64 * CH - 1;
  const double run = wave_last < G - 1 ? chunk_eval<MODEL, FDE, CH, false>(d, wc, c_over_H0, g0, lane, nu_pre, ln_pre, etab, dh, loc)
                                       : chunk_eval<MODEL, FDE, CH, true>(d, wc, c_over_H0, g0, lane, nu_pre, ln_pre, etab, dh, loc);
  const double incl = wave_inclusive_scan(run);
  const double first_dh = __hiloint2double(__builtin_amdgcn_readfirstlane(__double2hiint(dh[0])),
                                           __builtin_amdgcn_readfirstlane(__double2loint(dh[0])));
  if (lane == 63) wave_pub[wave] = (d4){incl, first_dh, dh[CH - 1], 0.0};
  __syncthreads();
  double term = 0.0;
  if (lane < CF_TPB_A / 64) {
    const d4 pv = wave_pub[lane];
    term = lane < wave ? pv[0] : 0.0;
    if (lane >= 1) {
      const int gb = lane * 64 * CH;
      const double zb = gb == G - 1 ? d.z_max : (double)gb * d.step;
      const double bnd = (wave_pub[lane - 1][2] + pv[1]) / 2 * (zb - (double)(gb - 1) * d.step);
      term += (lane <= wave && gb < G) ? bnd : 0.0;
    }
  }
  term += dpp_move<0x111, 0xF>(term);
  term += dpp_move<0x112, 0xF>(term);
  term += dpp_move<0x114, 0xF>(term);
  const double carry = (incl - run) + __hiloint2double(__builtin_amdgcn_readlane(__double2hiint(term), 7),
                                                       __builtin_amdgcn_readlane(__double2loint(term), 7));
#pragma unroll
  for (int k = 0; k < CH; ++k)
    if (g0 + k < G) tab[base + k] = (d2){loc[k] + carry, dh[k]};
  if (tid > 0 && g0 < G) tab[base - 1] = (d2){loc[0] + carry, dh[0]};
  __syncthreads();
}

template <int MODEL, int FDE>
__device__ __forceinline__ void build_distance_table_lds(const cf_dev_desc& d, const WalkerCosmo& wc, d2* tab,
                                                         d4* wave_pub) {
  double* wave_tot = reinterpret_cast<double*>(wave_pub);
  const int G = d.n_grid, chs = d.chunk_shift, CH = 1 << chs;
  const int tid = threadIdx.x, lane = tid & 63, wave = tid >> 6;
  const int g0 = tid << chs;
  const int base = g0 + tid;
  const int n_own = max(0, min(CH, G - g0));
  const double c_over_H0 = wc.c / wc.H0;
  for (int k = 0; k < n_own; ++k)
    tab[base + k].y = dh_of_node<MODEL, FDE>(d, wc, c_over_H0, g0 + k);
  __syncthreads();
  double run = 0.0;
  double prev = g0 > 0 && n_own > 0 ? tab[base - 2].y : 0.0;
  for (int k = 0; k < n_own; ++k) {
    const int g = g0 + k;
    const double cur = tab[base + k].y;
    if (g >= 1) {
      const double dz = grid_z(g, G, d.step, d.z_max) - grid_z(g - 1, G, d.step, d.z_max);
      run += (prev + cur) / 2 * dz;
    }
    tab[base + k].x = run;
    prev = cur;
  }
  const double incl = wave_inclusive_scan(run);
  if (lane == 63) wave_tot[wave] = incl;
  __syncthreads();
  double carry = incl - run;
  for (int w = 0; w < wave; ++w) carry += wave_tot[w];
  for (int k = 0; k < n_own; ++k) tab[base + k].x += carry;
  if (tid > 0 && n_own > 0) tab[base - 1] = tab[base];
  __syncthreads();
}

template <int MODEL, int FDE>
__device__ __forceinline__ void build_distance_table(const cf_dev_desc& d, const WalkerCosmo& wc, d2* tab,
                                                     d4* wave_pub, const double (&nu_pre)[8], const double (&ln_pre)[8],
                                                     const double* __restrict__ etab) {
  if (d.chunk_shift == 3) build_distance_table_regs<MODEL, FDE, 8>(d, wc, tab, wave_pub, nu_pre, ln_pre, etab);
  else build_distance_table_lds<MODEL, FDE>(d, wc, tab, wave_pub);
}

__device__ __forceinline__ double sgn_d(double v) { return (double)((v > 0) - (v < 0)); }

template <class TAB>
__device__ double pchip_slope_tab(const TAB& T, int i) {
  const int n = T.G;
  auto X = [&](int k) { return grid_z(k, n, T.step, T.z_max); };
  auto Y = [&](int k) { return T.at(k).y; };
  if (i > 0 && i < n - 1) {
    const double hl = X(i) - X(i - 1), hr = X(i + 1) - X(i);
    const double dl = (Y(i) - Y(i - 1)) / hl, dr = (Y(i + 1) - Y(i)) / hr;
    if (dl != 0.0 && dr != 0.0 && dl * dr > 0.0) {
      const double w1 = 2.0 * hr + hl, w2 = hr + 2.0 * hl;
      return (w1 + w2) / (w1 / dl + w2 / dr);
    }
    return 0.0;
  }
  double h0, h1, d0, d1;
  if (i == 0) {
    h0 = X(1) - X(0); h1 = X(2) - X(1);
    d0 = (Y(1) - Y(0)) / h0; d1 = (Y(2) - Y(1)) / h1;
  } else {
    h0 = X(n - 1) - X(n - 2); h1 = X(n - 2) - X(n - 3);
    d0 = (Y(n - 1) - Y(n - 2)) / h0; d1 = (Y(n - 2) - Y(n - 3)) / h1;
  }
  const double e = ((2 * h0 + h1) * d0 - h0 * d1) / (h0 + h1);
  if (d0 == 0.0 || sgn_d(e) != sgn_d(d0)) return 0.0;
  if (sgn_d(d0) != sgn_d(d1) && fabs(e) > fabs(3 * d0)) return 3 * d0;
  return e;
}

template <class TAB>
__device__ double pchip_dh_tab(const TAB& T, double xi) {
  const int G = T.G;
  if (xi <= 0.0) return T.at(0).y;
  if (xi >= T.z_max) return T.at(G - 1).y;
  int i = (int)(xi * T.inv_step);
  i = i > G - 2 ? G - 2 : i;
  if (i > 0 && grid_z(i, G, T.step, T.z_max) >= xi) --i;
  if (i < G - 2 && grid_z(i + 1, G, T.step, T.z_max) < xi) ++i;
  const double x0 = grid_z(i, G, T.step, T.z_max);
  const double h_i = grid_z(i + 1, G, T.step, T.z_max) - x0;
  const double t = (xi - x0) / h_i;
  const double t2 = t * t, t3 = t2 * t;
  const double h00 = 2 * t3 - 3 * t2 + 1, h10 = t3 - 2 * t2 + t, h01 = -2 * t3 + 3 * t2, h11 = t3 - t2;
  return h00 * T.at(i).y + h10 * h_i * pchip_slope_tab(T, i) + h01 * T.at(i + 1).y + h11 * h_i * pchip_slope_tab(T, i + 1);
}

__device__ double z_star_fit(const double* f, double wb, double wm) {
  wb = pow(wb, f[2]);
  wm = pow(wm, f[3]);
  return pow(wm, f[4]) + f[0] * f[5] * pow(wb, f[6]) * pow(wm, f[7]) + f[1] * f[8] * pow(wm, f[9]) * pow(wb, f[10]);
}
__device__ double r_drag_fit(const double* f, double wb, double wm) {
  wb = pow(wb, f[0]);
  wm = pow(wm, f[1]);
  const double den = (f[2] * pow(wb, f[3])) + (f[4] * pow(wb, f[5]) * pow(wm, f[6])) + (f[7] * pow(wm, f[8]));
  return 1.0 / den - f[9] / pow(wm, f[10]);
}

template <bool FRAG>
__device__ __forceinline__ int delta_index(int i) {
  return FRAG ? ((i >> 3) * 128 + ((i >> 1) & 3) * 32 + (i & 1)) : i;
}
template <bool PM1, bool LIN = false, bool FRAG = false, class D = cf_dev_desc>
__device__ __forceinline__ void sn_fast_loop(const D& d, const DistTable& T, const d2* __restrict__ log_tab,
                                             double* __restrict__ out, double off, double v100, int tid, double lin = 0.0,
                                             int part = 0, int n_parts = 1) {
  const int n_sn = d.n_sn, first = part * CF_TPB_A + tid, stride = n_parts * CF_TPB_A;
  double r_pos = 1.0, r_neg = 1.0, c0 = 0.0;
  if (PM1 && d.has_vstep) {
    r_pos = 1.0 / (1.0 + v100 / d.c);
    r_neg = 1.0 / (1.0 + (-v100) / d.c);
    c0 = -1.0;
  }
  const d4* __restrict__ rec = reinterpret_cast<const d4*>(d.sn_rec) + first;
  if (part == 0 && tid < d.n_ld - n_sn) out[delta_index<FRAG>(n_sn + tid)] = 0.0;
  auto one_sn = [&](const d4& r, int i) {
    const double za = r[0], st = r[1], zhp1 = r[2], ob = r[3];
    double z_cosmo = za;
    if (!LIN && PM1) {
      z_cosmo = fma(za, st > 0.0 ? r_pos : r_neg, c0);
    } else if (!LIN && d.has_vstep) {
      const double z_pec = (v100 * st) / d.c;
      z_cosmo = -1.0 + za / (1.0 + z_pec);
    }
    const double off_i = LIN ? off + lin * st : off;
    out[delta_index<FRAG>(i)] = ob - off_i - fma_vsv(log10_tab(zhp1 * hermite_fast(T, z_cosmo), log_tab), 5.0, 25.0);
  };
  d4 ra = rec[0], rb;
  int i = first;
  while (i < n_sn) {
    rb = rec[stride];
    one_sn(ra, i);
    i += stride;
    if (i >= n_sn) break;
    rec += 2 * stride;
    ra = rec[0];
    one_sn(rb, i);
    i += stride;
  }
}

template <int MODEL, int FDE>
__global__ void __launch_bounds__(CF_TPB_A, 4)
walker_kernel(cf_dev_desc d, const double* __restrict__ theta, int64_t W, double* __restrict__ delta,
              double* __restrict__ dm_out, double* __restrict__ mucorr_out, d2* __restrict__ bao_nodes, d2* __restrict__ table_out) {
  extern __shared__ __align__(16) d2 lds_tab[];
  __shared__ __align__(16) d4 wave_pub[CF_TPB_A / 64];
  __shared__ __align__(16) d2 log_tab[64];
  __shared__ double exp2_tab[64];

  const int64_t w = blockIdx.x;
  if (w >= W) return;
  const double* th = theta + w * d.ndim;
  const int tid = threadIdx.x;
  if (tid < 64 && d.n_sn > 0) log_tab[tid] = reinterpret_cast<const d2*>(d.log10_tab)[tid];
  double nu_pre[8], ln_pre[8];
  constexpr bool POWER_LAW = FDE == CF_FDE_WCDM_D || FDE == CF_FDE_CPL_D;
#pragma unroll
  for (int k = 0; k < 8; ++k) {
    nu_pre[k] = (MODEL == CF_EZ_PHYSICAL_D && d.chunk_shift == 3) ? d.nu_sw[k * CF_TPB_A + tid] : -1.0;
    ln_pre[k] = (POWER_LAW && d.chunk_shift == 3) ? d.ln_sw[k * CF_TPB_A + tid] : -1.0;
  }
  if (POWER_LAW && d.chunk_shift == 3 && tid >= 64 && tid < 128) exp2_tab[tid - 64] = d.exp2_tab[tid - 64];
  if (POWER_LAW && d.chunk_shift == 3) __syncthreads();
  const WalkerCosmo wc = make_cosmo(d, th);
  DistTable T;
  T.tab = lds_tab;
  T.G = d.n_grid;
  T.chs = d.chunk_shift;
  T.step = d.step;
  T.inv_step = d.inv_step;
  T.inv_last = d.inv_last;
  T.z_max = d.z_max;
  if (d.n_sn > 0 || d.n_aux > 0 || table_out) build_distance_table<MODEL, FDE>(d, wc, lds_tab, wave_pub, nu_pre, ln_pre, exp2_tab);
  if (table_out)
    for (int g = tid; g < d.n_grid; g += CF_TPB_A) table_out[w * d.n_grid + g] = T.at(g);
  for (int e = CF_TPB_A - 1 - tid; e < CF_BAO_NODES * d.n_aux; e += CF_TPB_A) {
    const int k = e / CF_BAO_NODES, o = e % CF_BAO_NODES;
    bao_nodes[(w * d.n_aux + k) * CF_BAO_NODES + o] = T.at(d.bao_base[k] + o);
  }

  if (d.n_sn > 0) {
    double* out = delta + w * d.n_ld;
    const double off = slot_get(d, CF_P_OFFSET_D, th);
    const double v100 = 100 * slot_get(d, CF_P_V_D, th);
    const double lin = d.sn_lin ? slot_get(d, CF_P_LIN_D, th) : 0.0;
    const bool parts = dm_out != nullptr || mucorr_out != nullptr;
    if (!parts && !d.sn_fixed_mu && !d.sn_dir && !d.sn_vel_mult && (!d.sn_lin || d.lin_in_rec)) {
      if (d.lin_in_rec) sn_fast_loop<false, true>(d, T, log_tab, out, off, v100, tid, lin);
      else if (d.step_pm1) sn_fast_loop<true>(d, T, log_tab, out, off, v100, tid);
      else sn_fast_loop<false>(d, T, log_tab, out, off, v100, tid);
    } else {
      const double vx = slot_get(d, CF_P_V_D, th), vy = slot_get(d, CF_P_V2_D, th), vz = slot_get(d, CF_P_V3_D, th);
      for (int i = tid; i < d.n_ld; i += CF_TPB_A) {
        double res = 0.0;
        if (i < d.n_sn) {
          const double zc = d.z_cmb[i];
          const double off_i = d.sn_lin ? off + lin * d.sn_lin[i] : off;
          double z_cosmo = zc;
          if (d.has_vstep) {
            const double v_km_s = d.sn_dir ? 100 * (d.sn_dir[3 * i] * vx + d.sn_dir[3 * i + 1] * vy + d.sn_dir[3 * i + 2] * vz) * d.sn_step[i]
                                           : v100 * d.sn_step[i];
            const double z_pec = v_km_s / d.c;
            z_cosmo = -1.0 + (1.0 + zc) / (1.0 + z_pec);
            if (d.sn_vel_mult) z_cosmo = fmax((1.0 + zc) * (1.0 + z_pec) - 1.0, 1e-8);
          }
          const double DMc = hermite_tab(T, z_cosmo);
          const double fixed = d.sn_fixed_mu ? d.sn_fixed_mu[i] : __longlong_as_double(0x7ff8000000000000ll);
          if (fixed == fixed) {
            const double DM = hermite_tab(T, zc);
            const double mu_corr = d.has_vstep ? 5.0 * log10_pos(DMc / DM) : 0.0;
            res = d.obs[i] - off_i - mu_corr - fixed;
            if (dm_out) dm_out[w * d.n_sn + i] = DM;
            if (mucorr_out) mucorr_out[w * d.n_sn + i] = mu_corr;
          } else if (!parts) {
            res = d.obs[i] - off_i - (25.0 + 5 * log10_pos((1.0 + d.z_hel[i]) * DMc));
          } else {
            const double DM = hermite_tab(T, zc);
            const double mu_corr = d.has_vstep ? 5.0 * log10(DMc / DM) : 0.0;
            const double mu_th = 25.0 + 5 * log10((1.0 + d.z_hel[i]) * DM);
            res = d.obs[i] - off_i - mu_corr - mu_th;
            if (dm_out) dm_out[w * d.n_sn + i] = DM;
            if (mucorr_out) mucorr_out[w * d.n_sn + i] = mu_corr;
          }
        }
        out[i] = res;
      }
    }
  }
}

template <int MODEL, int FDE>
__global__ void __launch_bounds__(CF_TPB_A, 4)
walker_fast_kernel(cf_walker_args d, const double* __restrict__ theta, int64_t W, double* __restrict__ delta,
                   d2* __restrict__ bao_nodes, double* __restrict__ theta_copy, int frag_b, int sn_parts) {
  extern __shared__ __align__(16) d2 lds_tab[];
  __shared__ __align__(16) d4 wave_pub[CF_TPB_A / 64];
  __shared__ __align__(16) d2 log_tab[64];
  __shared__ double exp2_all[CF_TPB_A / 64][64];

  const int64_t w = sn_parts > 1 ? blockIdx.x / (unsigned)sn_parts : blockIdx.x;
  const int part = sn_parts > 1 ? (int)(blockIdx.x % (unsigned)sn_parts) : 0;
  if (w >= W) return;
  const int tid = threadIdx.x, lane = tid & 63;
  double* const exp2_tab = exp2_all[tid >> 6];
  const ThetaRow th{theta[w * d.ndim + (lane < d.ndim ? lane : 0)]};
  if (theta_copy && part == 0 && tid < d.ndim) theta_copy[w * d.ndim + tid] = th.v;
  constexpr bool POWER_LAW = FDE == CF_FDE_WCDM_D || FDE == CF_FDE_CPL_D;
  d2 lt = (d2){0.0, 0.0};
  double et = 0.0;
  if (tid < 64 && d.n_sn > 0) lt = reinterpret_cast<const d2*>(d.log10_tab)[tid];
  if (POWER_LAW) et = d.exp2_tab[lane];
  double nu_pre[8], ln_pre[8];
#pragma unroll
  for (int k = 0; k < 8; ++k) {
    nu_pre[k] = MODEL == CF_EZ_PHYSICAL_D ? d.nu_sw[k * CF_TPB_A + tid] : -1.0;
    ln_pre[k] = POWER_LAW ? d.ln_sw[k * CF_TPB_A + tid] : -1.0;
  }
  if (tid < 64 && d.n_sn > 0) log_tab[tid] = lt;
  if (POWER_LAW) exp2_tab[lane] = et;
  const WalkerCosmo wc = make_cosmo(d, th);
  const double off = slot_get(d, CF_P_OFFSET_D, th);
  const double v100 = 100 * slot_get(d, CF_P_V_D, th);
  const double lin = d.lin_in_rec ? slot_get(d, CF_P_LIN_D, th) : 0.0;
  DistTable T;
  T.tab = lds_tab;
  T.G = d.n_grid;
  T.chs = 3;
  T.step = d.step;
  T.inv_step = d.inv_step;
  T.inv_last = d.inv_last;
  T.z_max = d.z_max;
  build_distance_table_regs<MODEL, FDE, 8>(d, wc, lds_tab, wave_pub, nu_pre, ln_pre, exp2_tab);
  for (int e = CF_TPB_A - 1 - tid; part == 0 && e < CF_BAO_NODES * d.n_aux; e += CF_TPB_A) {
    const int k = e / CF_BAO_NODES, o = e % CF_BAO_NODES;
    bao_nodes[(w * d.n_aux + k) * CF_BAO_NODES + o] = T.at(d.bao_base[k] + o);
  }
  if (d.n_sn > 0 && !frag_b) {
    double* out = delta + w * d.n_ld;
    if (d.lin_in_rec) sn_fast_loop<false, true>(d, T, log_tab, out, off, v100, tid, lin, part, sn_parts);
    else if (d.step_pm1) sn_fast_loop<true>(d, T, log_tab, out, off, v100, tid, 0.0, part, sn_parts);
    else sn_fast_loop<false>(d, T, log_tab, out, off, v100, tid, 0.0, part, sn_parts);
  } else if (d.n_sn > 0) {
    double* out = delta + (w >> 4) * (16 * (int64_t)d.n_ld) + 2 * (w & 15);
    if (d.lin_in_rec) sn_fast_loop<false, true, true>(d, T, log_tab, out, off, v100, tid, lin, part, sn_parts);
    else if (d.step_pm1) sn_fast_loop<true, false, true>(d, T, log_tab, out, off, v100, tid, 0.0, part, sn_parts);
    else sn_fast_loop<false, false, true>(d, T, log_tab, out, off, v100, tid, 0.0, part, sn_parts);
  }
}

template <int MODEL, int FDE>
__device__ __forceinline__ double H_at_gl_node(const cf_dev_desc& d, const WalkerCosmo& wc, double z, const double* __restrict__ etab,
                                               const d2* __restrict__ ltab) {
  const double zp1 = 1.0 + z;
  const double cubed = zp1 * zp1 * zp1;
  double f = 1.0;
  if (FDE == CF_FDE_WCDM_D) {
    f = exp_tab((3 * (1 + wc.w0)) * (log10_tab(zp1, ltab) * 2.30258509299404568402), etab);
  } else if (FDE == CF_FDE_CPL_D) {
    f = exp_tab(fma(3 * (1 + wc.w0 + wc.wa), log10_tab(zp1, ltab) * 2.30258509299404568402, div_pos(-3 * wc.wa * z, zp1)), etab);
  } else if (FDE == CF_FDE_THAWING_D) {
    const double r = div_pos(2 * cubed, (1.0 + wc.w0) + (1.0 - wc.w0) * cubed);
    f = r * r;
  }
  double e2;
  if (MODEL == CF_EZ_LATE_FLAT_D) {
    e2 = (FDE == CF_FDE_LCDM_D) ? wc.Om * cubed + (1.0 - wc.Om) : wc.Om * cubed + (1.0 - wc.Om) * f;
  } else {
    const double de = (FDE == CF_FDE_LCDM_D) ? wc.Ode : wc.Ode * f;
    const double r = div_pos(d.nu_m0, zp1), mz_sq = r * r;
    const double ws = sqrt_pos(d.nu_qs_sq[0] + mz_sq) * d.nu_ws[0] + sqrt_pos(d.nu_qs_sq[1] + mz_sq) * d.nu_ws[1] +
                      sqrt_pos(d.nu_qs_sq[2] + mz_sq) * d.nu_ws[2] + sqrt_pos(d.nu_qs_sq[3] + mz_sq) * d.nu_ws[3] +
                      sqrt_pos(d.nu_qs_sq[4] + mz_sq) * d.nu_ws[4];
    const double zp1_2 = zp1 * zp1;
    const double nu = div_pos(zp1_2 * zp1_2 * ws, d.nu_rho0);
    e2 = wc.Or * (cubed * zp1) + wc.Obc * cubed + de + wc.Onu * nu;
  }
  return wc.H0 * sqrt_pos(e2);
}

template <int LANES>
__device__ __forceinline__ double group_sum(double v) {
#pragma unroll
  for (int o = LANES / 2; o >= 1; o >>= 1) v += __shfl_xor(v, o, LANES);
  return v;
}

template <int LANES>
struct VirtualLaneSum {
  static constexpr int NV = 64 / LANES;
  double a[NV];
  __device__ __forceinline__ VirtualLaneSum() {
#pragma unroll
    for (int j = 0; j < NV; ++j) a[j] = 0.0;
  }
  __device__ __forceinline__ void push(double t) {
    const double tmp = a[0] + t;
#pragma unroll
    for (int j = 0; j + 1 < NV; ++j) a[j] = a[j + 1];
    a[NV - 1] = tmp;
  }
  __device__ __forceinline__ double total(int pushes) const {
    double v[NV];
#pragma unroll
    for (int j = 0; j < NV; ++j) {
      v[j] = a[0];
#pragma unroll
      for (int i = 1; i < NV; ++i) v[j] = (((j - pushes) & (NV - 1)) == i) ? a[i] : v[j];
    }
    double r = v[0];
    if (NV == 2) r = v[0] + v[1];
    if (NV == 4) r = (v[0] + v[2]) + (v[1] + v[3]);
    return group_sum<LANES>(r);
  }
};

template <int LANES>
__device__ __forceinline__ double group_quadratic_form(const double* __restrict__ dl, const double* __restrict__ inv_cov, int n,
                                                       int sl) {
  VirtualLaneSum<LANES> acc;
  const int iters = (n + LANES - 1) / LANES;
  for (int it = 0; it < iters; ++it) {
    const int j = sl + it * LANES, jc = j < n ? j : n - 1;
    double t = 0.0;
    for (int i0 = 0; i0 < n; i0 += 8) {
      double c[8];
#pragma unroll
      for (int k = 0; k < 8; ++k) c[k] = inv_cov[(i0 + k < n ? i0 + k : n - 1) * n + jc];
#pragma unroll
      for (int k = 0; k < 8; ++k)
// ... 370 lines not shown
    if (lane >= dlt) P = mm(P, R);
  }
  if (lane == 63) wave_tot[wave] = P;
  __syncthreads();
  M22 E = shfl_up_m(P, 1);
  if (lane == 0) E = M22{1.0, 0.0, 0.0, 1.0};
  for (int v = wave - 1; v >= 0; --v) E = mm(E, wave_tot[v]);

  double y1 = E.a * d.fs8_a_init + E.b, y2 = E.c * d.fs8_a_init + E.d;
#pragma unroll
  for (int j = 0; j < C; ++j) {
    bnd[C * tid + j] = d2{y2, s_at[j] * y1 - p_at[j] * y2};
    const double n1 = M[j].a * y1 + M[j].b * y2, n2 = M[j].c * y1 + M[j].d * y2;
    y1 = n1;
    y2 = n2;
  }
  if (tid == CF_GROWTH_TPB - 1) {
    bnd[S] = d2{y2, s_end * y1 - p_end * y2};
    resid[CF_MAX_FS8] = y1;
  }
  __syncthreads();

  const double delta0 = resid[CF_MAX_FS8], s8 = slot_get(d, CF_P_S8_D, th), ferr = slot_get(d, CF_P_FS8ERR_D, th);
  if (wave == 0 && lane < n) {
    const int k = d.fs8_order[lane], i = d.fs8_step_of[lane];
    const d4* pt = reinterpret_cast<const d4*>(d.fs8_pts) + 8 * lane;
    const d4 hw = pt[0], aux = pt[1];
    auto read_out = [&](const d4& wgt, int step) {
      const d2 b0 = bnd[step], b1 = bnd[step + 1];
      return wgt[0] * b0[0] + wgt[1] * b0[1] + wgt[2] * b1[0] + wgt[3] * b1[1];
    };
    double dprime;
    if (d.fs8_n_agrid > 0) {
      const d4 xs = pt[6], st = pt[7];
      const double y0 = read_out(pt[2], (int)st[0]), y1 = read_out(pt[3], (int)st[1]), y2 = read_out(pt[4], (int)st[2]),
                   y3 = read_out(pt[5], (int)st[3]);
      dprime = pchip_window4(xs[0], xs[1], xs[2], xs[3], y0, y1, y2, y3, (int)aux[2], (int)aux[3], aux[0]);
    } else {
      dprime = read_out(hw, i);
    }
    NodeView T;
    T.p = aux_nodes + (w * d.n_aux + d.n_bao + k) * CF_BAO_NODES;
    T.base = d.bao_base[d.n_bao + k];
    T.G = d.n_grid; T.step = d.step; T.inv_step = d.inv_step; T.inv_last = d.inv_last; T.z_max = d.z_max;
    const double z = d.fs8_z[k];
    const double theory = (s8 / delta0) * aux[0] * dprime;
    const double Hz = wc.H0 * sqrt(e2_of_z<MODEL, FDE>(d, wc, z, MODEL == CF_EZ_PHYSICAL_D ? aux[1] : -1.0));
    const double q = Hz * hermite_tab(T, z) / d.fs8_fid[k];
    if (theory_out) theory_out[w * n + k] = theory;
    resid[k] = d.fs8_val[k] - theory / q;
  }
  __syncthreads();
  double tj = 0.0;
  if (lane < n) {
    const double* col = d.fs8_inv_cov + lane;
#pragma unroll 4
    for (int i = wave; i < n; i += 4) tj += resid[i] * col[i * n];
  }
  part[wave * 64 + lane] = tj;
  __syncthreads();
  if (wave != 0) return;
  double r_own = lane < n ? (((part[lane] + part[64 + lane]) + part[128 + lane]) + part[192 + lane]) * resid[lane] : 0.0;
#pragma unroll
  for (int off = 32; off > 0; off >>= 1) r_own += __shfl_xor(r_own, off);
  if (lane == 0) {
    const double c = r_own * (ferr * ferr);
    chi2_extra[w] = accumulate ? chi2_extra[w] + c : c;
    if (blocks_out) blocks_out[w] = c;
  }
}

template <int MODEL, int FDE>
__global__ void hz_kernel(cf_dev_desc d, const double* __restrict__ theta, const double* __restrict__ z, int64_t n,
                          double* __restrict__ out) {
  const int64_t i = blockIdx.x * (int64_t)blockDim.x + threadIdx.x;
  if (i >= n) return;
  const WalkerCosmo wc = make_cosmo(d, theta);
  out[i] = H_of_z<MODEL, FDE>(d, wc, z[i]);
}

#define CF_INSTANTIATE_GROWTH(M, F, C) \
  template __global__ void growth_kernel<M, F, C>(cf_dev_desc, const double*, int64_t, const d2*, double*, int, double*, double*);
#define CF_INSTANTIATE_WALKER(M, F)                                                                              \
  template __global__ void walker_kernel<M, F>(cf_dev_desc, const double*, int64_t, double*, double*, double*, d2*, d2*); \
  template __global__ void walker_fast_kernel<M, F>(cf_walker_args, const double*, int64_t, double*, d2*, double*, int, int);     \
  template __global__ void small_blocks_kernel<M, F, 16, 1>(cf_dev_desc, const double*, int64_t, const d2*, double*, double*, \
                                                            double*);                                                      \
  template __global__ void small_blocks_kernel<M, F, 64, 1>(cf_dev_desc, const double*, int64_t, const d2*, double*, double*, \
                                                            double*);                                                      \
  template __global__ void small_blocks_kernel<M, F, 64, 2>(cf_dev_desc, const double*, int64_t, const d2*, double*, double*, \
                                                            double*);                                                      \
  template __global__ void hz_kernel<M, F>(cf_dev_desc, const double*, const double*, int64_t, double*);                     \
  CF_INSTANTIATE_GROWTH(M, F, 1) CF_INSTANTIATE_GROWTH(M, F, 2) CF_INSTANTIATE_GROWTH(M, F, 4) CF_INSTANTIATE_GROWTH(M, F, 8)
CF_INSTANTIATE_WALKER(0, 0) CF_INSTANTIATE_WALKER(0, 1) CF_INSTANTIATE_WALKER(0, 2) CF_INSTANTIATE_WALKER(0, 3)
CF_INSTANTIATE_WALKER(1, 0) CF_INSTANTIATE_WALKER(1, 1) CF_INSTANTIATE_WALKER(1, 2) CF_INSTANTIATE_WALKER(1, 3)

__device__ __forceinline__ double epi_slot(const cf_dev_slot& sl, const double* __restrict__ th) {
  return sl.idx >= 0 ? th[sl.idx] * sl.scale : sl.fixed;
}
__device__ __forceinline__ double finalize_value(const cf_epilogue& d, const double* __restrict__ th, double chi2, int out_kind,
                                                 unsigned long long* nonfinite) {
  for (int g = 0; g < d.n_chi2_gauss; ++g) {
    double diff = th[d.chi2_gauss_idx[g]] - d.chi2_gauss_mean[g];
    chi2 += diff * diff / (d.chi2_gauss_sigma[g] * d.chi2_gauss_sigma[g]);
  }
  if (out_kind == CF_OUT_CHI2_D) return chi2;
  double lp = 0.0;
  if (out_kind == CF_OUT_LOGP_D) {
    if (d.has_bounds) {
      bool inbox = true;
      for (int k0 = 0; k0 < d.ndim; k0 += 4) {
#pragma unroll
        for (int k = k0; k < k0 + 4; ++k) {
          const double t = th[k < d.ndim ? k : 0];
          inbox = inbox & ((k >= d.ndim) | ((d.lo[k & (CF_MAX_NDIM - 1)] < t) & (t < d.hi[k & (CF_MAX_NDIM - 1)])));
        }
      }
      if (!inbox) return -INFINITY;
      lp = d.log_norm;
    }
    for (int g = 0; g < d.n_gauss; ++g) {
      double diff = th[d.gauss_idx[g]] - d.gauss_mean[g];
      lp = lp - 0.5 * (diff * diff) / (d.gauss_sigma[g] * d.gauss_sigma[g]);
    }
  }
  if (d.cpl_wall && epi_slot(d.w0, th) + epi_slot(d.wa, th) >= 0.0) return lp + -1e8;
  if (!isfinite(chi2)) {
    atomicAdd(nonfinite, 1ull);
    return -INFINITY;
  }
  double ll = -0.5 * chi2 + d.logl_const;
  if (d.n_fs8 > 0)
    ll += d.n_fs8 * log(epi_slot(d.fs8err, th));
  if (d.n_cc > 0)
    ll -= 0.5 * (d.n_cc * 1.8378770664093453 + d.cc_logdet +
                 (d.cc_f_inverse ? 2 : -2) * d.n_cc * log(epi_slot(d.fcc, th)));
  return lp + ll;
}


__device__ __forceinline__ d4 mfma_f64(double a, double b, d4 c) {
  return __builtin_amdgcn_mfma_f64_16x16x4f64(a, b, c, 0, 0, 0);
}

template <int NT, int PF, int NTU>
__device__ __forceinline__ void update_loop(d4 (&acc)[NTU], const d2* __restrict__ A, const d2* __restrict__ Yp,
                                            int n_s2, int lane) {
  d2 a[PF][NT];
  d2 yb[PF];
  const d2* Ap = A + lane;
  const d2* Yq = Yp + lane;
  __builtin_amdgcn_sched_barrier(0);
#pragma unroll
  for (int p = 0; p < PF; ++p) {
#pragma unroll
    for (int j = 0; j < NT; ++j) a[p][j] = Ap[(p * NT + j) * 64];
    yb[p] = Yq[p * 64];
    __builtin_amdgcn_sched_barrier(0);
  }
  Ap += PF * NT * 64;
  Yq += PF * 64;
  for (int s2 = 0; s2 < n_s2; s2 += PF) {
#pragma unroll
    for (int p = 0; p < PF; ++p) {
#pragma unroll
      for (int j = 0; j < NT; ++j) acc[j] = mfma_f64(a[p][j].x, yb[p].x, acc[j]);
#pragma unroll
      for (int j = 0; j < NT; ++j) acc[j] = mfma_f64(a[p][j].y, yb[p].y, acc[j]);
// ... 754 lines not shown
```

include/cosmofit.h:

```cpp
#ifndef COSMOFIT_H
#define COSMOFIT_H

#include <stdint.h>

#ifdef __cplusplus
extern "C" {
#endif

#define CF_ABI_VERSION 11

typedef struct cf_handle cf_handle;

enum cf_status {
  CF_OK = 0,
  CF_ERR_INVALID = -1,
  CF_ERR_NO_DEVICE = -2,
  CF_ERR_HIP = -3,
  CF_ERR_NOT_POSDEF = -4,
  CF_ERR_UNSUPPORTED = -5,
  CF_ERR_ILL_CONDITIONED = -6
};

enum cf_ez_model {
  CF_EZ_LATE_FLAT = 0,
// ... 100 lines not shown
  int32_t rd_mode;
  int32_t _pad1;
  const double* bao_z;
  const double* bao_val;
  const int32_t* bao_qty;
  const double* bao_inv_cov;
  double rd_fit[11];

  int32_t cmb_mode;
  int32_t n_gl;
  const double* gl_x;
  const double* gl_w;
  double cmb_prior[3];
  double cmb_inv_cov[9];
  double zstar_fit[11];
  double o_gamma_h2;

  double or_h2;
  double omnu_h2;
  double nu_m0;
  double nu_rho0;
  double nu_qs_sq[5];
  double nu_ws[5];

  const double* bounds;
  int32_t n_gauss;
  int32_t cpl_wall;
  const cf_gauss_prior* gauss;
  int32_t n_chi2_gauss;
  int32_t _pad2;
  const cf_gauss_prior* chi2_gauss;

  const double* sn_fixed_mu;

  int32_t n_cc;
  int32_t _pad3;
  const double* cc_z;
  const double* cc_h;
  const double* cc_inv_cov;
  double cc_logdet;

  int32_t solve_mode;
  int32_t _pad4;
  double probe_limit;

  int32_t n_devices;
  int32_t _pad5;
  const int32_t* devices;

  int32_t om_mode;
  int32_t rd_wm_mode;
  const double* sn_lin_coef;
  const double* sn_dir;

  int32_t n_fs8;
  int32_t fs8_steps;
  const double* fs8_z;
  const double* fs8_val;
  const double* fs8_inv_cov;
  const double* fs8_fid;
  double logl_const;
  double fs8_a_init;

  int32_t sn_vel_mode;
  int32_t cc_f_mode;
  int32_t prior_norm_mode;
  int32_t fs8_n_agrid;
} cf_desc;

typedef struct cf_info {
  int64_t n_sn;
  int64_t n_sn_pad;
  int64_t packed_chol_bytes;
  int64_t workspace_bytes;
  int64_t max_walkers;
  int64_t nonfinite_count;
  int32_t device;
  int32_t cu_count;
  char gcn_arch[64];
  double pack_probe_rel;
  int32_t solve_mode;
  int32_t n_devices;
  int32_t devices[16];
} cf_info;

int cf_device_count(void);
const char* cf_last_error(void);
int cf_abi_version(void);

int cf_create(const cf_desc* desc, cf_handle** out);
void cf_destroy(cf_handle* h);
int cf_get_info(cf_handle* h, cf_info* info);

int cf_eval(cf_handle* h, const double* theta, int64_t W, double* out, int32_t out_kind);

void cf_split_rows(int64_t W, int32_t n, int32_t k, int64_t* begin, int64_t* end);

int cf_eval_device(cf_handle* h, const double* d_theta, int64_t W, double* d_out,
                   int32_t out_kind, void* hip_stream);

int cf_eval_parts(cf_handle* h, const double* theta, int64_t W, double* dm_obs, double* mu_corr,
                  double* delta, double* chi2_blocks, double* bao_theory, double* fs8_theory);

int cf_eval_table(cf_handle* h, const double* theta, int64_t W, double* cum_dm, double* dh);

int cf_eval_bao_at(cf_handle* h, const double* theta, const double* z, const int32_t* qty, int64_t n, double* out);

int cf_eval_hz(cf_handle* h, const double* theta, const double* z, int64_t n, double* out);

int cf_eval_fs8_at(cf_handle* h, const double* theta, const double* z, int64_t n, double* out);

int cf_enable_timing(cf_handle* h, int slots);
int cf_set_timing_stride(cf_handle* h, int stride);
int64_t cf_timed_calls(cf_handle* h);
int cf_kernel_ms(cf_handle* h, int64_t call, float t[2]);
int cf_kernel_ms3(cf_handle* h, int64_t call, float t[3]);
int cf_last_kernel_ms(cf_handle* h, float t[2]);

int cf_interp_hermite(const double* xq, int64_t nq, const double* x, const double* y,
                      const double* y_prime, int64_t n, double* out);
int cf_interp_pchip(const double* xq, int64_t nq, const double* x, const double* y, int64_t n,
                    double* out);
int cf_solve_triangular(const double* L, int64_t n, int64_t ld, const double* b, int64_t nrhs,
                        double* out);

int cf_selftest_pack_host(const double* L, int64_t n, int64_t ld, const double* b, double* chi2_out,
                          int64_t* packed_bytes);

int cf_selftest_invpack_host(const double* L, int64_t n, int64_t ld, const double* b, double* chi2_out,
                             double* probe_out);

int cf_selftest_log10(const double* x, int64_t n, double* out);
int cf_selftest_log10_tab(const double* x, int64_t n, double* out);
int cf_selftest_exp_tab(const double* x, int64_t n, double* out);
int cf_selftest_pos_ops(const double* a, const double* b, int64_t n, double* out);

int64_t cf_ens_active_count(uint64_t split_key, int32_t n_splits, int32_t split, int64_t shard_start, int64_t shard_stop);
int64_t cf_ens_comp_count(uint64_t split_key, int32_t n_splits, int32_t split, int64_t w_total);
int cf_ens_active_set(uint64_t split_key, int32_t n_splits, int32_t split, int64_t shard_start, int64_t shard_stop,
                      int64_t* d_ids, int64_t* d_local_idx, void* hip_stream);
int cf_ens_kde_prepare(const double* d_all_pos, int64_t w_total, int32_t ndim, int32_t n_splits, int32_t split,
                       uint64_t split_key, double* d_params, double* d_wc, void* hip_stream);
int cf_ens_propose(int32_t kind, const double* d_all_pos, int64_t w_total, int32_t ndim, int32_t n_splits, int32_t split,
                   uint64_t split_key, const int64_t* d_ids, int64_t n_active, uint64_t key0, double a, double de_sigma,
                   const double* d_kde_params, const double* d_kde_wc, double* d_y, double* d_log_factor,
                   void* hip_stream);
int cf_ens_accept(const int64_t* d_ids, const int64_t* d_local_idx, int64_t n_active, int32_t ndim, uint64_t key0,
                  const double* d_y, const double* d_lp_new, const double* d_log_factor, double* d_x_local,
                  double* d_logp_local, uint64_t* d_n_accepted, void* hip_stream);
int cf_ens_accept_record(const int64_t* d_ids, const int64_t* d_local_idx, int64_t n_active, int32_t ndim, uint64_t key0,
                         const double* d_y, const double* d_lp_new, const double* d_log_factor, double* d_x_local,
                         double* d_logp_local, uint64_t* d_n_accepted, double* d_chain_slot, double* d_logp_slot,
                         int64_t* d_walker_accepted, void* hip_stream);

int cf_chain_mean(const double* d_x, int64_t n_t, int64_t n_s, double* d_mean, void* hip_stream);
int cf_chain_lagsum(const double* d_x, const double* d_mean, int64_t n_t, int64_t n_s, int64_t lag0, int32_t nlag,
                    double* d_out, void* hip_stream);
int cf_chain_acf_mean(const double* d_lagsum, const double* d_c0, int64_t n_w, int32_t ndim, int32_t nlag, double* d_f,
                      void* hip_stream);

#define CF_MARG_MAX_NDIM 16
#define CF_MARG_MAX_BINS 128
#define CF_MARG_MAX_PAIRS 256
#define CF_MARG_MAX_SEGMENTS 65536
#define CF_MARG_NOT_COUNTED 255
int cf_marg_bin(const double* d_x, int64_t n, int32_t ndim, const double* d_edges, int32_t nbins, uint8_t* d_idx,
// ... 259 lines not shown
```

Before: 18.05 million evals/s.

## Template walker kernels on block size and add a 256-thread variant

Walker and fast-walker kernels are now templated on threads-per-block, so each thread handles a chunk size of 4096/TPB grid nodes, with matching node swizzling, LDS padding shift and launch bounds. A 256-thread variant with 16-node chunks and a tail-handling scheme in chunk_eval is added, selectable via the CF_TUNE walker_tpb key. The default stays at 512, so the default path is mostly the same kernel restructured, with small tail-masking and Hermite-lookup refactors. The larger variant trades more per-thread register work for fewer threads and fewer cross-wave scan steps.

```diff
diff --git a/cosmology-model-fit_amd/_lib.py b/cosmology-model-fit_amd/_lib.py
--- a/cosmology-model-fit_amd/_lib.py
+++ b/cosmology-model-fit_amd/_lib.py
@@ -192,7 +192,7 @@
         ("workspace_bytes", C.c_int64), ("max_walkers", C.c_int64), ("nonfinite_count", C.c_int64),
         ("device", C.c_int32), ("cu_count", C.c_int32), ("gcn_arch", C.c_char * 64),
         ("pack_probe_rel", C.c_double), ("solve_mode", C.c_int32), ("n_devices", C.c_int32),
-        ("devices", C.c_int32 * 16),
+        ("devices", C.c_int32 * 16), ("walker_tpb", C.c_int32), ("reserved0", C.c_int32),
     ]
 
 
diff --git a/cosmology-model-fit_amd/csrc/cf_pack.h b/cosmology-model-fit_amd/csrc/cf_pack.h
--- a/cosmology-model-fit_amd/csrc/cf_pack.h
+++ b/cosmology-model-fit_amd/csrc/cf_pack.h
@@ -327,4 +327,16 @@
   return worst;
 }
 
+static inline std::vector<double> cf_swizzle_nodes(const std::vector<double>& table, int tpb) {
+  const int ch = 4096 / tpb;
+  std::vector<double> out((size_t)4096);
+  const size_t n = table.size();
+  for (int k = 0; k < ch; ++k)
+    for (int t = 0; t < tpb; ++t) {
+      const size_t g = (size_t)ch * t + k;
+      out[(size_t)k * tpb + t] = table[g < n - 1 ? g : n - 1];
+    }
+  return out;
+}
+
 #endif
diff --git a/cosmology-model-fit_amd/csrc/cosmofit_api.hip b/cosmology-model-fit_amd/csrc/cosmofit_api.hip
--- a/cosmology-model-fit_amd/csrc/cosmofit_api.hip
+++ b/cosmology-model-fit_amd/csrc/cosmofit_api.hip
@@ -41,10 +41,10 @@
 #define CF_BAO_NODES 6
 #define CF_SN_PARTS_MAX 4
 #define CF_SN_REC_SLACK (512 * CF_SN_PARTS_MAX)
-template <int MODEL, int FDE>
+template <int MODEL, int FDE, int TPB>
 __global__ void walker_kernel(cf_dev_desc d, const double* theta, int64_t W, double* delta, double* dm_out, double* mucorr_out,
                               d2* bao_nodes, d2* table_out);
-template <int MODEL, int FDE>
+template <int MODEL, int FDE, int TPB>
 __global__ void walker_fast_kernel(cf_walker_args d, const double* theta, int64_t W, double* delta, d2* bao_nodes, double* theta_copy,
                                    int frag_b, int sn_parts);
 template <int MODEL, int FDE, int LANES, int ROLES>
@@ -58,8 +58,10 @@
 #define CF_DECLARE_GROWTH(M, F, C) \
   extern template __global__ void growth_kernel<M, F, C>(cf_dev_desc, const double*, int64_t, const d2*, double*, int, double*, double*);
 #define CF_DECLARE_WALKER(M, F)                                                                                            \
-  extern template __global__ void walker_kernel<M, F>(cf_dev_desc, const double*, int64_t, double*, double*, double*, d2*, d2*); \
-  extern template __global__ void walker_fast_kernel<M, F>(cf_walker_args, const double*, int64_t, double*, d2*, double*, int, int); \
+  extern template __global__ void walker_kernel<M, F, 512>(cf_dev_desc, const double*, int64_t, double*, double*, double*, d2*, d2*); \
+  extern template __global__ void walker_kernel<M, F, 256>(cf_dev_desc, const double*, int64_t, double*, double*, double*, d2*, d2*); \
+  extern template __global__ void walker_fast_kernel<M, F, 512>(cf_walker_args, const double*, int64_t, double*, d2*, double*, int, int); \
+  extern template __global__ void walker_fast_kernel<M, F, 256>(cf_walker_args, const double*, int64_t, double*, d2*, double*, int, int); \
   extern template __global__ void small_blocks_kernel<M, F, 16, 1>(cf_dev_desc, const double*, int64_t, const d2*, double*, \
                                                                    double*, double*);                                      \
   extern template __global__ void small_blocks_kernel<M, F, 64, 1>(cf_dev_desc, const double*, int64_t, const d2*, double*, \
@@ -71,19 +73,33 @@
 CF_DECLARE_WALKER(0, 0) CF_DECLARE_WALKER(0, 1) CF_DECLARE_WALKER(0, 2) CF_DECLARE_WALKER(0, 3)
 CF_DECLARE_WALKER(1, 0) CF_DECLARE_WALKER(1, 1) CF_DECLARE_WALKER(1, 2) CF_DECLARE_WALKER(1, 3)
 
+#ifndef CF_DEFAULT_WALKER_TPB
+#define CF_DEFAULT_WALKER_TPB 512
+#endif
+static int walker_tpb_env() {
+  static const int tpb = [] {
+    const long long v = cf_tune("walker_tpb", CF_DEFAULT_WALKER_TPB);
+    return v == 256 || v == 512 ? (int)v : CF_DEFAULT_WALKER_TPB;
+  }();
+  return tpb;
+}
+static int walker_tpb_of(const cf_dev_desc& d) { return d.chunk_shift == 3 ? walker_tpb_env() : 512; }
+static size_t walker_lds_of(const cf_dev_desc& d) {
+  const int chs = walker_tpb_of(d) == 256 ? 4 : d.chunk_shift;
+  return ((size_t)d.n_grid + (d.n_grid >> chs) + 2) * 16;
+}
 typedef void (*walker_fn)(cf_dev_desc, const double*, int64_t, double*, double*, double*, d2*, d2*);
-static walker_fn pick_walker(int model, int fde) {
-  static const walker_fn table[2][4] = {
-      {walker_kernel<0, 0>, walker_kernel<0, 1>, walker_kernel<0, 2>, walker_kernel<0, 3>},
-      {walker_kernel<1, 0>, walker_kernel<1, 1>, walker_kernel<1, 2>, walker_kernel<1, 3>}};
-  return table[model][fde];
+static walker_fn pick_walker(int model, int fde, int tpb) {
+#define CF_WALKER_TABLE(K, T) \
+  {{K<0, 0, T>, K<0, 1, T>, K<0, 2, T>, K<0, 3, T>}, {K<1, 0, T>, K<1, 1, T>, K<1, 2, T>, K<1, 3, T>}}
+  static const walker_fn table[2][2][4] = {CF_WALKER_TABLE(walker_kernel, 512), CF_WALKER_TABLE(walker_kernel, 256)};
+  return table[tpb == 256][model][fde];
 }
 typedef void (*walker_fast_fn)(cf_walker_args, const double*, int64_t, double*, d2*, double*, int, int);
-static walker_fast_fn pick_walker_fast(int model, int fde) {
-  static const walker_fast_fn table[2][4] = {
-      {walker_fast_kernel<0, 0>, walker_fast_kernel<0, 1>, walker_fast_kernel<0, 2>, walker_fast_kernel<0, 3>},
-      {walker_fast_kernel<1, 0>, walker_fast_kernel<1, 1>, walker_fast_kernel<1, 2>, walker_fast_kernel<1, 3>}};
-  return table[model][fde];
+static walker_fast_fn pick_walker_fast(int model, int fde, int tpb) {
+  static const walker_fast_fn table[2][2][4] = {CF_WALKER_TABLE(walker_fast_kernel, 512), CF_WALKER_TABLE(walker_fast_kernel, 256)};
+  return table[tpb == 256][model][fde];
+#undef CF_WALKER_TABLE
 }
 static bool walker_fast_ok(const cf_dev_desc& d) {
   static const bool off = cf_tune("walker_generic", 0) != 0;
@@ -379,14 +395,6 @@
   return b < 0 ? 0 : (b > G - CF_BAO_NODES ? G - CF_BAO_NODES : b);
 }
 
-static std::vector<double> swizzle_for_walker_threads(const std::vector<double>& table) {
-  std::vector<double> out(8 * 512);
-  const size_t n = table.size();
-  for (int k = 0; k < 8; ++k)
-    for (int t = 0; t < 512; ++t) out[(size_t)k * 512 + t] = table[std::min((size_t)(8 * t + k), n - 1)];
-  return out;
-}
-
 static int upload_vec(DevBuf& b, const double* src, int64_t n) {
   if (b.ensure((size_t)n * 8)) return CF_ERR_HIP;
   HIP_TRY(hipMemcpy(b.p, src, (size_t)n * 8, hipMemcpyHostToDevice));
@@ -901,7 +909,7 @@
     if ((rc = upload_vec(h->nu_grid, nu.data(), c->n_grid))) return bail(rc);
     d.nu_grid = h->nu_grid.as<const double>();
     if (d.chunk_shift == 3) {
-      const std::vector<double> sw = swizzle_for_walker_threads(nu);
+      const std::vector<double> sw = cf_swizzle_nodes(nu, walker_tpb_of(d));
       if ((rc = upload_vec(h->nu_sw, sw.data(), (int64_t)sw.size()))) return bail(rc);
       d.nu_sw = h->nu_sw.as<const double>();
     }
@@ -916,7 +924,7 @@
     if ((rc = upload_vec(h->ln_grid, ln.data(), c->n_grid))) return bail(rc);
     d.ln_grid = h->ln_grid.as<const double>();
     if (d.chunk_shift == 3) {
-      const std::vector<double> sw = swizzle_for_walker_threads(ln);
+      const std::vector<double> sw = cf_swizzle_nodes(ln, walker_tpb_of(d));
       if ((rc = upload_vec(h->ln_sw, sw.data(), (int64_t)sw.size()))) return bail(rc);
       d.ln_sw = h->ln_sw.as<const double>();
       if ((rc = upload_exp2_table(h->exp2_tab))) return bail(rc);
@@ -1066,6 +1074,7 @@
   info->cu_count = h->cu_count;
   info->pack_probe_rel = h->pack_probe_rel;
   info->n_devices = 1 + (int32_t)h->peers.size();
+  info->walker_tpb = walker_tpb_of(h->d);
   info->devices[0] = h->device;
   for (size_t k = 0; k < h->peers.size() && k + 1 < 16; ++k) info->devices[k + 1] = h->peers[k]->device;
   snprintf(info->gcn_arch, sizeof(info->gcn_arch), "%s", h->arch);
@@ -1265,17 +1274,18 @@
     if (th_copy) th = th_copy;
     if (ev) HIP_TRY(hipEventRecord(ev[1], st));
   } else if (walker_work) {
-    const size_t lds = ((size_t)d.n_grid + (d.n_grid >> d.chunk_shift) + 2) * 16;
+    const size_t lds = walker_lds_of(d);
+    const int tpb = walker_tpb_of(d);
     if (!dm_out && !mucorr_out && walker_fast_ok(d)) {
       double* th_copy = h->theta_on_host ? h->theta.as<double>() : nullptr;
       static const int parts_env = (int)cf_tune("sn_parts", 0);
       int sn_parts = parts_env > 0 ? parts_env : (Wc <= 64 ? 4 : (Wc <= 160 ? 2 : 1));
       if (sn_parts > CF_SN_PARTS_MAX || d.n_sn == 0) sn_parts = 1;
-      hipLaunchKernelGGL(pick_walker_fast(d.ez_model, d.fde), dim3((unsigned)(Wc * sn_parts)), dim3(512), lds, st, walker_args_of(d), th,
+      hipLaunchKernelGGL(pick_walker_fast(d.ez_model, d.fde, tpb), dim3((unsigned)(Wc * sn_parts)), dim3(tpb), lds, st, walker_args_of(d), th,
                          Wc, delta, bao_nodes, th_copy, frag_b ? 1 : 0, sn_parts);
       if (th_copy) th = th_copy;
     } else
-      hipLaunchKernelGGL(pick_walker(d.ez_model, d.fde), dim3((unsigned)Wc), dim3(512), lds, st, d, th, Wc, delta, dm_out, mucorr_out,
+      hipLaunchKernelGGL(pick_walker(d.ez_model, d.fde, tpb), dim3((unsigned)Wc), dim3(tpb), lds, st, d, th, Wc, delta, dm_out, mucorr_out,
                          bao_nodes, (d2*)nullptr);
     if (ev) HIP_TRY(hipEventRecord(ev[1], st));
     if (h->has_small_blocks) {
@@ -1558,8 +1568,8 @@
   DevBuf tab;
   if (tab.ensure((size_t)W * G * sizeof(d2))) return CF_ERR_HIP;
   HIP_TRY(hipMemcpyAsync(h->theta.p, theta, (size_t)W * d.ndim * 8, hipMemcpyHostToDevice, h->stream));
-  const size_t lds = ((size_t)G + (G >> d.chunk_shift) + 2) * 16;
-  hipLaunchKernelGGL(pick_walker(d.ez_model, d.fde), dim3((unsigned)W), dim3(512), lds, h->stream, d, h->theta.as<const double>(), W,
+  const size_t lds = walker_lds_of(d);
+  hipLaunchKernelGGL(pick_walker(d.ez_model, d.fde, walker_tpb_of(d)), dim3((unsigned)W), dim3(walker_tpb_of(d)), lds, h->stream, d, h->theta.as<const double>(), W,
                      (double*)nullptr, (double*)nullptr, (double*)nullptr, (d2*)nullptr, tab.as<d2>());
   HIP_TRY(hipGetLastError());
   std::vector<cf_d2> host((size_t)W * G);
@@ -1614,8 +1624,8 @@
     d.fs8_z = dz.as<const double>(); d.bao_base = dbase.as<const int32_t>(); d.fs8_step_of = dstep.as<const int32_t>();
     d.fs8_order = dorder.as<const int32_t>(); d.fs8_pts = dpts.as<const double>(); d.fs8_val = dval.as<const double>();
     d.fs8_inv_cov = dinv.as<const double>(); d.fs8_fid = dfid.as<const double>();
-    const size_t lds = ((size_t)d.n_grid + (d.n_grid >> d.chunk_shift) + 2) * 16;
-    hipLaunchKernelGGL(pick_walker(d.ez_model, d.fde), dim3(1), dim3(512), lds, h->stream, d, h->theta.as<const double>(), (int64_t)1,
+    const size_t lds = walker_lds_of(d);
+    hipLaunchKernelGGL(pick_walker(d.ez_model, d.fde, walker_tpb_of(d)), dim3(1), dim3(walker_tpb_of(d)), lds, h->stream, d, h->theta.as<const double>(), (int64_t)1,
                        (double*)nullptr, (double*)nullptr, (double*)nullptr, nodes.as<d2>(), (d2*)nullptr);
     hipLaunchKernelGGL(pick_growth(d.ez_model, d.fde, d.fs8_steps), dim3(1), dim3(256),
                        (size_t)(2 * (d.fs8_steps + 1) + 16 + CF_MAX_FS8 + 2 + 256) * 8, h->stream, d, h->theta.as<const double>(),
@@ -1685,8 +1695,8 @@
     HIP_TRY(hipMemcpyAsync(dbase.p, base.data(), (size_t)m * 4, hipMemcpyHostToDevice, h->stream));
     d.bao_z = dz.as<const double>(); d.bao_qty = dq.as<const int32_t>(); d.bao_base = dbase.as<const int32_t>();
     d.bao_val = dval.as<const double>(); d.bao_inv_cov = dinv.as<const double>();
-    const size_t lds = ((size_t)d.n_grid + (d.n_grid >> d.chunk_shift) + 2) * 16;
-    hipLaunchKernelGGL(pick_walker(d.ez_model, d.fde), dim3(1), dim3(512), lds, h->stream, d, h->theta.as<const double>(), (int64_t)1,
+    const size_t lds = walker_lds_of(d);
+    hipLaunchKernelGGL(pick_walker(d.ez_model, d.fde, walker_tpb_of(d)), dim3(1), dim3(walker_tpb_of(d)), lds, h->stream, d, h->theta.as<const double>(), (int64_t)1,
                        (double*)nullptr, (double*)nullptr, (double*)nullptr, nodes.as<d2>(), (d2*)nullptr);
     hipLaunchKernelGGL(pick_small_blocks(d.ez_model, d.fde, 16), dim3(1), dim3(256), 0, h->stream, d, h->theta.as<const double>(), (int64_t)1,
                        (const d2*)nodes.as<d2>(), extra.as<double>(), (double*)nullptr, dout.as<double>());
diff --git a/cosmology-model-fit_amd/csrc/cosmofit_kernels.hip b/cosmology-model-fit_amd/csrc/cosmofit_kernels.hip
--- a/cosmology-model-fit_amd/csrc/cosmofit_kernels.hip
+++ b/cosmology-model-fit_amd/csrc/cosmofit_kernels.hip
@@ -248,21 +248,26 @@
   return r;
 }
 
+template <bool ANY>
+__device__ __forceinline__ double hermite_fast_cubic(const DistTable& T, double xi) {
+  const int G = T.G;
+  const double u = xi * T.inv_step;
+  int i = (int)u;
+  i = i > G - 2 ? G - 2 : i;
+  if (ANY) i = i < 0 ? 0 : i;
+  const double t = u - (double)i;
+  const d2* p = T.tab + (i + (i >> T.chs));
+  const d2 e0 = p[0], e1 = p[1];
+  const double b = T.step * e0.y, hm1 = T.step * e1.y, dy = e1.x - e0.x;
+  const double sm = b + hm1;
+  const double dd = fma(-2.0, dy, sm);
+  const double cc = fma(3.0, dy, -(sm + b));
+  return fma(t, fma(t, fma(t, dd, cc), b), e0.x);
+}
+
 __device__ __forceinline__ double hermite_fast(const DistTable& T, double xi) {
   const int G = T.G;
-  if (__builtin_expect(xi > 0.0 && xi < T.z_max, 1)) {
-    const double u = xi * T.inv_step;
-    int i = (int)u;
-    i = i > G - 2 ? G - 2 : i;
-    const double t = u - (double)i;
-    const d2* p = T.tab + (i + (i >> T.chs));
-    const d2 e0 = p[0], e1 = p[1];
-    const double b = T.step * e0.y, hm1 = T.step * e1.y, dy = e1.x - e0.x;
-    const double sm = b + hm1;
-    const double dd = fma(-2.0, dy, sm);
-    const double cc = fma(3.0, dy, -(sm + b));
-    return fma(t, fma(t, fma(t, dd, cc), b), e0.x);
-  }
+  if (__builtin_expect(xi > 0.0 && xi < T.z_max, 1)) return hermite_fast_cubic<false>(T, xi);
   if (xi <= 0.0) {
     const d2 e = T.at(0);
     return e.x + e.y * xi;
@@ -307,8 +312,10 @@
   return val_lo + ww;
 }
 
+__device__ __forceinline__ bool log10_tab_ok(double x) { return x > 2.2250738585072014e-308 && x < 1.7976931348623157e308; }
+template <bool RANGED = false>
 __device__ __forceinline__ double log10_tab(double x, const d2* __restrict__ tab) {
-  if (!(x > 2.2250738585072014e-308 && x < 1.7976931348623157e308)) return log10(x);
+  if (!RANGED && !log10_tab_ok(x)) return log10(x);
   const double C1 = 4.34294481903251827651e-01, C2 = -2.17147240951625913826e-01, C3 = 1.44764827301083942550e-01,
                C4 = -1.08573620475812956913e-01, C5 = 8.68588963806503655303e-02, C6 = -7.23824136505419712752e-02,
                C7 = 6.20420688433216896645e-02, C8 = -5.42868102379064784564e-02;
@@ -329,7 +336,7 @@
 }
 
 
-template <int MODEL, int FDE, int CH, bool LAST, class D>
+template <int MODEL, int FDE, int CH, int TAIL, class D>
 __device__ __forceinline__ double chunk_eval(const D& d, const WalkerCosmo& wc, double c_over_H0, int g0, int lane,
                                              const double (&nu_pre)[CH], const double (&ln)[CH], const double* __restrict__ etab,
                                              double (&dh)[CH], double (&loc)[CH]) {
@@ -342,7 +349,7 @@
     for (int k = 0; k < CH; ++k) {
       const int g = g0 + k;
       double z = (double)g * d.step;
-      if (LAST) z = g >= G - 1 ? d.z_max : z;
+      if (TAIL == 2 || (TAIL == 1 && k == CH - 1)) z = g >= G - 1 ? d.z_max : z;
       if (FDE == CF_FDE_CPL_D) {
         const double zp1 = 1.0 + z;
         double r = __builtin_amdgcn_rcp(zp1);
@@ -375,28 +382,30 @@
   for (int k = 0; k < CH; ++k) {
     const int g = g0 + k;
     double z = (double)g * d.step;
-    if (LAST) z = g >= G - 1 ? d.z_max : z;
+    if (TAIL == 2 || (TAIL == 1 && k == CH - 1)) z = g >= G - 1 ? d.z_max : z;
     const double e2 = POWER_LAW ? e2_from_fde<MODEL>(wc, z, fde[k], nu_pre[k]) : e2_of_z<MODEL, FDE, true, D>(d, wc, z, nu_pre[k], ln[k], etab);
-    const double v = c_over_H0 * rsqrt_pos(e2);
-    dh[k] = (LAST && g >= G) ? 0.0 : v;
+    dh[k] = c_over_H0 * rsqrt_pos(e2);
   }
   double prev = dpp_move<0x138, 0xF>(dh[CH - 1]);
   double run = 0.0;
   const double half = 0.5 * d.step;
 #pragma unroll
   for (int k = 0; k < CH; ++k) {
-    const bool counts = (k > 0 || lane > 0) && (!LAST || g0 + k < G);
-    run = counts ? fma_vsv(prev + dh[k], half, run) : run;
+    const bool counts = (k > 0 || lane > 0) && (TAIL == 0 || (TAIL == 1 ? k > 0 || g0 < G : g0 + k < G));
+    const double sum = counts ? prev + dh[k] : 0.0;
+    run = fma_vsv(sum, half, run);
     loc[k] = run;
     prev = dh[k];
   }
+  if (TAIL == 1) run = g0 < G ? run : 0.0;
   return run;
 }
 
-template <int MODEL, int FDE, int CH, class D>
+template <int MODEL, int FDE, int CH, int TPB, class D>
 __device__ __forceinline__ void build_distance_table_regs(const D& d, const WalkerCosmo& wc, d2* tab,
                                                           d4* wave_pub, const double (&nu_pre)[CH], const double (&ln_pre)[CH],
                                                           const double* __restrict__ etab) {
+  static_assert(CH * TPB == 4096 && (TPB == 512 || TPB == 256), "512 threads x 8 nodes or 256 threads x 16 nodes");
   const int G = d.n_grid;
   const int tid = threadIdx.x, lane = tid & 63, wave = tid >> 6;
   const int g0 = tid * CH;
@@ -404,15 +413,16 @@
   const double c_over_H0 = wc.c / wc.H0;
   double dh[CH], loc[CH];
   const int wave_last = (tid - lane) * CH + 64 * CH - 1;
-  const double run = wave_last < G - 1 ? chunk_eval<MODEL, FDE, CH, false>(d, wc, c_over_H0, g0, lane, nu_pre, ln_pre, etab, dh, loc)
-                                       : chunk_eval<MODEL, FDE, CH, true>(d, wc, c_over_H0, g0, lane, nu_pre, ln_pre, etab, dh, loc);
+  const double run = wave_last < G - 1    ? chunk_eval<MODEL, FDE, CH, 0>(d, wc, c_over_H0, g0, lane, nu_pre, ln_pre, etab, dh, loc)
+                     : (G & (CH - 1)) == 0 ? chunk_eval<MODEL, FDE, CH, 1>(d, wc, c_over_H0, g0, lane, nu_pre, ln_pre, etab, dh, loc)
+                                           : chunk_eval<MODEL, FDE, CH, 2>(d, wc, c_over_H0, g0, lane, nu_pre, ln_pre, etab, dh, loc);
   const double incl = wave_inclusive_scan(run);
   const double first_dh = __hiloint2double(__builtin_amdgcn_readfirstlane(__double2hiint(dh[0])),
                                            __builtin_amdgcn_readfirstlane(__double2loint(dh[0])));
   if (lane == 63) wave_pub[wave] = (d4){incl, first_dh, dh[CH - 1], 0.0};
   __syncthreads();
   double term = 0.0;
-  if (lane < CF_TPB_A / 64) {
+  if (lane < TPB / 64) {
     const d4 pv = wave_pub[lane];
     term = lane < wave ? pv[0] : 0.0;
     if (lane >= 1) {
@@ -469,12 +479,12 @@
   __syncthreads();
 }
 
-template <int MODEL, int FDE>
+template <int MODEL, int FDE, int TPB>
 __device__ __forceinline__ void build_distance_table(const cf_dev_desc& d, const WalkerCosmo& wc, d2* tab,
-                                                     d4* wave_pub, const double (&nu_pre)[8], const double (&ln_pre)[8],
+                                                     d4* wave_pub, const double (&nu_pre)[4096 / TPB], const double (&ln_pre)[4096 / TPB],
                                                      const double* __restrict__ etab) {
-  if (d.chunk_shift == 3) build_distance_table_regs<MODEL, FDE, 8>(d, wc, tab, wave_pub, nu_pre, ln_pre, etab);
-  else build_distance_table_lds<MODEL, FDE>(d, wc, tab, wave_pub);
+  if (d.chunk_shift == 3) build_distance_table_regs<MODEL, FDE, 4096 / TPB, TPB>(d, wc, tab, wave_pub, nu_pre, ln_pre, etab);
+  else if constexpr (TPB == CF_TPB_A) build_distance_table_lds<MODEL, FDE>(d, wc, tab, wave_pub);
 }
 
 __device__ __forceinline__ double sgn_d(double v) { return (double)((v > 0) - (v < 0)); }
@@ -540,11 +550,11 @@
 __device__ __forceinline__ int delta_index(int i) {
   return FRAG ? ((i >> 3) * 128 + ((i >> 1) & 3) * 32 + (i & 1)) : i;
 }
-template <bool PM1, bool LIN = false, bool FRAG = false, class D = cf_dev_desc>
+template <int TPB, bool PM1, bool LIN = false, bool FRAG = false, class D = cf_dev_desc>
 __device__ __forceinline__ void sn_fast_loop(const D& d, const DistTable& T, const d2* __restrict__ log_tab,
                                              double* __restrict__ out, double off, double v100, int tid, double lin = 0.0,
                                              int part = 0, int n_parts = 1) {
-  const int n_sn = d.n_sn, first = part * CF_TPB_A + tid, stride = n_parts * CF_TPB_A;
+  const int n_sn = d.n_sn, first = part * TPB + tid, stride = n_parts * TPB;
   double r_pos = 1.0, r_neg = 1.0, c0 = 0.0;
   if (PM1 && d.has_vstep) {
     r_pos = 1.0 / (1.0 + v100 / d.c);
@@ -553,8 +563,8 @@
   }
   const d4* __restrict__ rec = reinterpret_cast<const d4*>(d.sn_rec) + first;
   if (part == 0 && tid < d.n_ld - n_sn) out[delta_index<FRAG>(n_sn + tid)] = 0.0;
-  auto one_sn = [&](const d4& r, int i) {
-    const double za = r[0], st = r[1], zhp1 = r[2], ob = r[3];
+  auto z_cosmo_of = [&](const d4& r) {
+    const double za = r[0], st = r[1];
     double z_cosmo = za;
     if (!LIN && PM1) {
       z_cosmo = fma(za, st > 0.0 ? r_pos : r_neg, c0);
@@ -562,9 +572,50 @@
       const double z_pec = (v100 * st) / d.c;
       z_cosmo = -1.0 + za / (1.0 + z_pec);
     }
+    return z_cosmo;
+  };
+  auto one_sn = [&](const d4& r, int i) {
+    const double st = r[1], zhp1 = r[2], ob = r[3];
+    const double z_cosmo = z_cosmo_of(r);
     const double off_i = LIN ? off + lin * st : off;
     out[delta_index<FRAG>(i)] = ob - off_i - fma_vsv(log10_tab(zhp1 * hermite_fast(T, z_cosmo), log_tab), 5.0, 25.0);
   };
+  if constexpr (TPB == 256) {
+    auto two_sn = [&](const d4& r0, const d4& r1, int i) {
+      const double z0 = z_cosmo_of(r0), z1 = z_cosmo_of(r1);
+      const double x0 = r0[2] * hermite_fast_cubic<true>(T, z0), x1 = r1[2] * hermite_fast_cubic<true>(T, z1);
+      const double off0 = LIN ? off + lin * r0[1] : off, off1 = LIN ? off + lin * r1[1] : off;
+      const double res0 = r0[3] - off0 - fma_vsv(log10_tab<true>(x0, log_tab), 5.0, 25.0);
+      const double res1 = r1[3] - off1 - fma_vsv(log10_tab<true>(x1, log_tab), 5.0, 25.0);
+      const bool ok0 = z0 > 0.0 && z0 < T.z_max && log10_tab_ok(x0), ok1 = z1 > 0.0 && z1 < T.z_max && log10_tab_ok(x1);
+      if (ok0) out[delta_index<FRAG>(i)] = res0;
+      if (ok1) out[delta_index<FRAG>(i + stride)] = res1;
+      if (__builtin_expect(!ok0, 0)) one_sn(r0, i);
+      if (__builtin_expect(!ok1, 0)) one_sn(r1, i + stride);
+    };
+    if (first >= n_sn) return;
+    d4 ra = rec[0], rb = rec[stride];
+    for (int i = first;;) {
+      if (i + stride >= n_sn) {
+        one_sn(ra, i);
+        break;
+      }
+      const int i_next = i + 2 * stride;
+      const bool more = i_next < n_sn;
+      d4 na = ra, nb = rb;
+      if (more) {
+        na = rec[2 * stride];
+        nb = rec[3 * stride];
+      }
+      two_sn(ra, rb, i);
+      if (!more) break;
+      rec += 2 * stride;
+      ra = na;
+      rb = nb;
+      i = i_next;
+    }
+    return;
+  }
   d4 ra = rec[0], rb;
   int i = first;
   while (i < n_sn) {
@@ -579,12 +630,13 @@
   }
 }
 
-template <int MODEL, int FDE>
-__global__ void __launch_bounds__(CF_TPB_A, 4)
+template <int MODEL, int FDE, int TPB>
+__global__ void __launch_bounds__(TPB, TPB / 128)
 walker_kernel(cf_dev_desc d, const double* __restrict__ theta, int64_t W, double* __restrict__ delta,
               double* __restrict__ dm_out, double* __restrict__ mucorr_out, d2* __restrict__ bao_nodes, d2* __restrict__ table_out) {
+  constexpr int CH = 4096 / TPB;
   extern __shared__ __align__(16) d2 lds_tab[];
-  __shared__ __align__(16) d4 wave_pub[CF_TPB_A / 64];
+  __shared__ __align__(16) d4 wave_pub[TPB / 64];
   __shared__ __align__(16) d2 log_tab[64];
   __shared__ double exp2_tab[64];
 
@@ -593,12 +645,12 @@
   const double* th = theta + w * d.ndim;
   const int tid = threadIdx.x;
   if (tid < 64 && d.n_sn > 0) log_tab[tid] = reinterpret_cast<const d2*>(d.log10_tab)[tid];
-  double nu_pre[8], ln_pre[8];
+  double nu_pre[CH], ln_pre[CH];
   constexpr bool POWER_LAW = FDE == CF_FDE_WCDM_D || FDE == CF_FDE_CPL_D;
 #pragma unroll
-  for (int k = 0; k < 8; ++k) {
-    nu_pre[k] = (MODEL == CF_EZ_PHYSICAL_D && d.chunk_shift == 3) ? d.nu_sw[k * CF_TPB_A + tid] : -1.0;
-    ln_pre[k] = (POWER_LAW && d.chunk_shift == 3) ? d.ln_sw[k * CF_TPB_A + tid] : -1.0;
+  for (int k = 0; k < CH; ++k) {
+    nu_pre[k] = (MODEL == CF_EZ_PHYSICAL_D && d.chunk_shift == 3) ? d.nu_sw[k * TPB + tid] : -1.0;
+    ln_pre[k] = (POWER_LAW && d.chunk_shift == 3) ? d.ln_sw[k * TPB + tid] : -1.0;
   }
   if (POWER_LAW && d.chunk_shift == 3 && tid >= 64 && tid < 128) exp2_tab[tid - 64] = d.exp2_tab[tid - 64];
   if (POWER_LAW && d.chunk_shift == 3) __syncthreads();
@@ -606,15 +658,15 @@
   DistTable T;
   T.tab = lds_tab;
   T.G = d.n_grid;
-  T.chs = d.chunk_shift;
+  T.chs = TPB == CF_TPB_A ? d.chunk_shift : 4;
   T.step = d.step;
   T.inv_step = d.inv_step;
   T.inv_last = d.inv_last;
   T.z_max = d.z_max;
-  if (d.n_sn > 0 || d.n_aux > 0 || table_out) build_distance_table<MODEL, FDE>(d, wc, lds_tab, wave_pub, nu_pre, ln_pre, exp2_tab);
+  if (d.n_sn > 0 || d.n_aux > 0 || table_out) build_distance_table<MODEL, FDE, TPB>(d, wc, lds_tab, wave_pub, nu_pre, ln_pre, exp2_tab);
   if (table_out)
-    for (int g = tid; g < d.n_grid; g += CF_TPB_A) table_out[w * d.n_grid + g] = T.at(g);
-  for (int e = CF_TPB_A - 1 - tid; e < CF_BAO_NODES * d.n_aux; e += CF_TPB_A) {
+    for (int g = tid; g < d.n_grid; g += TPB) table_out[w * d.n_grid + g] = T.at(g);
+  for (int e = TPB - 1 - tid; e < CF_BAO_NODES * d.n_aux; e += TPB) {
     const int k = e / CF_BAO_NODES, o = e % CF_BAO_NODES;
     bao_nodes[(w * d.n_aux + k) * CF_BAO_NODES + o] = T.at(d.bao_base[k] + o);
   }
@@ -626,12 +678,12 @@
     const double lin = d.sn_lin ? slot_get(d, CF_P_LIN_D, th) : 0.0;
     const bool parts = dm_out != nullptr || mucorr_out != nullptr;
     if (!parts && !d.sn_fixed_mu && !d.sn_dir && !d.sn_vel_mult && (!d.sn_lin || d.lin_in_rec)) {
-      if (d.lin_in_rec) sn_fast_loop<false, true>(d, T, log_tab, out, off, v100, tid, lin);
-      else if (d.step_pm1) sn_fast_loop<true>(d, T, log_tab, out, off, v100, tid);
-      else sn_fast_loop<false>(d, T, log_tab, out, off, v100, tid);
+      if (d.lin_in_rec) sn_fast_loop<TPB, false, true>(d, T, log_tab, out, off, v100, tid, lin);
+      else if (d.step_pm1) sn_fast_loop<TPB, true>(d, T, log_tab, out, off, v100, tid);
+      else sn_fast_loop<TPB, false>(d, T, log_tab, out, off, v100, tid);
     } else {
       const double vx = slot_get(d, CF_P_V_D, th), vy = slot_get(d, CF_P_V2_D, th), vz = slot_get(d, CF_P_V3_D, th);
-      for (int i = tid; i < d.n_ld; i += CF_TPB_A) {
+      for (int i = tid; i < d.n_ld; i += TPB) {
         double res = 0.0;
         if (i < d.n_sn) {
           const double zc = d.z_cmb[i];
@@ -669,14 +721,15 @@
   }
 }
 
-template <int MODEL, int FDE>
-__global__ void __launch_bounds__(CF_TPB_A, 4)
+template <int MODEL, int FDE, int TPB>
+__global__ void __launch_bounds__(TPB, TPB / 128)
 walker_fast_kernel(cf_walker_args d, const double* __restrict__ theta, int64_t W, double* __restrict__ delta,
                    d2* __restrict__ bao_nodes, double* __restrict__ theta_copy, int frag_b, int sn_parts) {
+  constexpr int CH = 4096 / TPB;
   extern __shared__ __align__(16) d2 lds_tab[];
-  __shared__ __align__(16) d4 wave_pub[CF_TPB_A / 64];
+  __shared__ __align__(16) d4 wave_pub[TPB / 64];
   __shared__ __align__(16) d2 log_tab[64];
-  __shared__ double exp2_all[CF_TPB_A / 64][64];
+  __shared__ double exp2_all[TPB / 64][64];
 
   const int64_t w = sn_parts > 1 ? blockIdx.x / (unsigned)sn_parts : blockIdx.x;
   const int part = sn_parts > 1 ? (int)(blockIdx.x % (unsigned)sn_parts) : 0;
@@ -690,11 +743,11 @@
   double et = 0.0;
   if (tid < 64 && d.n_sn > 0) lt = reinterpret_cast<const d2*>(d.log10_tab)[tid];
   if (POWER_LAW) et = d.exp2_tab[lane];
-  double nu_pre[8], ln_pre[8];
-#pragma unroll
-  for (int k = 0; k < 8; ++k) {
-    nu_pre[k] = MODEL == CF_EZ_PHYSICAL_D ? d.nu_sw[k * CF_TPB_A + tid] : -1.0;
-    ln_pre[k] = POWER_LAW ? d.ln_sw[k * CF_TPB_A + tid] : -1.0;
+  double nu_pre[CH], ln_pre[CH];
+#pragma unroll
+  for (int k = 0; k < CH; ++k) {
+    nu_pre[k] = MODEL == CF_EZ_PHYSICAL_D ? d.nu_sw[k * TPB + tid] : -1.0;
+    ln_pre[k] = POWER_LAW ? d.ln_sw[k * TPB + tid] : -1.0;
   }
   if (tid < 64 && d.n_sn > 0) log_tab[tid] = lt;
   if (POWER_LAW) exp2_tab[lane] = et;
@@ -705,26 +758,26 @@
   DistTable T;
   T.tab = lds_tab;
   T.G = d.n_grid;
-  T.chs = 3;
+  T.chs = TPB == CF_TPB_A ? 3 : 4;
   T.step = d.step;
   T.inv_step = d.inv_step;
   T.inv_last = d.inv_last;
   T.z_max = d.z_max;
-  build_distance_table_regs<MODEL, FDE, 8>(d, wc, lds_tab, wave_pub, nu_pre, ln_pre, exp2_tab);
-  for (int e = CF_TPB_A - 1 - tid; part == 0 && e < CF_BAO_NODES * d.n_aux; e += CF_TPB_A) {
+  build_distance_table_regs<MODEL, FDE, CH, TPB>(d, wc, lds_tab, wave_pub, nu_pre, ln_pre, exp2_tab);
+  for (int e = TPB - 1 - tid; part == 0 && e < CF_BAO_NODES * d.n_aux; e += TPB) {
     const int k = e / CF_BAO_NODES, o = e % CF_BAO_NODES;
     bao_nodes[(w * d.n_aux + k) * CF_BAO_NODES + o] = T.at(d.bao_base[k] + o);
   }
   if (d.n_sn > 0 && !frag_b) {
     double* out = delta + w * d.n_ld;
-    if (d.lin_in_rec) sn_fast_loop<false, true>(d, T, log_tab, out, off, v100, tid, lin, part, sn_parts);
-    else if (d.step_pm1) sn_fast_loop<true>(d, T, log_tab, out, off, v100, tid, 0.0, part, sn_parts);
-    else sn_fast_loop<false>(d, T, log_tab, out, off, v100, tid, 0.0, part, sn_parts);
+    if (d.lin_in_rec) sn_fast_loop<TPB, false, true>(d, T, log_tab, out, off, v100, tid, lin, part, sn_parts);
+    else if (d.step_pm1) sn_fast_loop<TPB, true>(d, T, log_tab, out, off, v100, tid, 0.0, part, sn_parts);
+    else sn_fast_loop<TPB, false>(d, T, log_tab, out, off, v100, tid, 0.0, part, sn_parts);
   } else if (d.n_sn > 0) {
     double* out = delta + (w >> 4) * (16 * (int64_t)d.n_ld) + 2 * (w & 15);
-    if (d.lin_in_rec) sn_fast_loop<false, true, true>(d, T, log_tab, out, off, v100, tid, lin, part, sn_parts);
-    else if (d.step_pm1) sn_fast_loop<true, false, true>(d, T, log_tab, out, off, v100, tid, 0.0, part, sn_parts);
-    else sn_fast_loop<false, false, true>(d, T, log_tab, out, off, v100, tid, 0.0, part, sn_parts);
+    if (d.lin_in_rec) sn_fast_loop<TPB, false, true, true>(d, T, log_tab, out, off, v100, tid, lin, part, sn_parts);
+    else if (d.step_pm1) sn_fast_loop<TPB, true, false, true>(d, T, log_tab, out, off, v100, tid, 0.0, part, sn_parts);
+    else sn_fast_loop<TPB, false, false, true>(d, T, log_tab, out, off, v100, tid, 0.0, part, sn_parts);
   }
 }
 
@@ -1261,8 +1314,10 @@
 #define CF_INSTANTIATE_GROWTH(M, F, C) \
   template __global__ void growth_kernel<M, F, C>(cf_dev_desc, const double*, int64_t, const d2*, double*, int, double*, double*);
 #define CF_INSTANTIATE_WALKER(M, F)                                                                              \
-  template __global__ void walker_kernel<M, F>(cf_dev_desc, const double*, int64_t, double*, double*, double*, d2*, d2*); \
-  template __global__ void walker_fast_kernel<M, F>(cf_walker_args, const double*, int64_t, double*, d2*, double*, int, int);     \
+  template __global__ void walker_kernel<M, F, 512>(cf_dev_desc, const double*, int64_t, double*, double*, double*, d2*, d2*); \
+  template __global__ void walker_kernel<M, F, 256>(cf_dev_desc, const double*, int64_t, double*, double*, double*, d2*, d2*); \
+  template __global__ void walker_fast_kernel<M, F, 512>(cf_walker_args, const double*, int64_t, double*, d2*, double*, int, int); \
+  template __global__ void walker_fast_kernel<M, F, 256>(cf_walker_args, const double*, int64_t, double*, d2*, double*, int, int); \
   template __global__ void small_blocks_kernel<M, F, 16, 1>(cf_dev_desc, const double*, int64_t, const d2*, double*, double*, \
                                                             double*);                                                      \
   template __global__ void small_blocks_kernel<M, F, 64, 1>(cf_dev_desc, const double*, int64_t, const d2*, double*, double*, \
diff --git a/include/cosmofit.h b/include/cosmofit.h
--- a/include/cosmofit.h
+++ b/include/cosmofit.h
@@ -206,6 +206,8 @@
   int32_t solve_mode;
   int32_t n_devices;
   int32_t devices[16];
+  int32_t walker_tpb;
+  int32_t reserved0;
 } cf_info;
 
 int cf_device_count(void);
```

New measurement: 18.09 million evals/s (median of 5 runs). No clear change (+0.2%).
